# JakobHavtorn/benchmarking-lvms

Measured on AMD Instinct MI355X. Metric: audio frames/sec training (VRNN, 16 kHz mu-law), higher is better.
Workload: dtype f32

## Files before the change

### benchmarking-lvms_amd/csrc/pchain.h

```cpp
#pragma once
#include <algorithm>
#include <cstdlib>

#include "common.h"

namespace blvm {
namespace pchain {

constexpr unsigned SENTINEL = 0xFFFFFFFFu;
constexpr unsigned SPIN_LIMIT = 1u << 22;

typedef unsigned u32x4 __attribute__((ext_vector_type(4)));
typedef __amdgpu_buffer_rsrc_t rsrc_t;
constexpr int AUX_SC1 = 16;
#ifndef PCHAIN_POLL_AUX
#define PCHAIN_POLL_AUX AUX_SC1
#endif
#ifndef PCHAIN_STORE_AUX
#define PCHAIN_STORE_AUX AUX_SC1
#endif
__device__ __forceinline__ rsrc_t make_rsrc(const void* base) {
  const unsigned long long u = reinterpret_cast<unsigned long long>(base);
  const unsigned lo = (unsigned)__builtin_amdgcn_readfirstlane((int)(unsigned)u), hi = (unsigned)__builtin_amdgcn_readfirstlane((int)(unsigned)(u >> 32));
  return __builtin_amdgcn_make_buffer_rsrc(reinterpret_cast<void*>(((unsigned long long)hi << 32) | lo), 0, 0xFFFFFFFFu, 0x00020000);
}
__device__ __forceinline__ f32x4 ld_sc1_x4(rsrc_t r, unsigned byte_off) {
  return __builtin_bit_cast(f32x4, __builtin_amdgcn_raw_buffer_load_b128(r, (int)byte_off, 0, PCHAIN_POLL_AUX));
}
__device__ __forceinline__ float ld_sc1(rsrc_t r, unsigned byte_off) {
  return __builtin_bit_cast(float, __builtin_amdgcn_raw_buffer_load_b32(r, (int)byte_off, 0, PCHAIN_POLL_AUX));
}
__device__ __forceinline__ void st_sc1(rsrc_t r, unsigned byte_off, float v) {
  __builtin_amdgcn_raw_buffer_store_b32(__builtin_bit_cast(unsigned, v), r, (int)byte_off, 0, PCHAIN_STORE_AUX);
}

__device__ __forceinline__ bool is_sentinel(float x) { return __float_as_uint(x) == SENTINEL; }
__device__ __forceinline__ bool any_sentinel(const f32x4& v) {
  return is_sentinel(v[0]) | is_sentinel(v[1]) | is_sentinel(v[2]) | is_sentinel(v[3]);
}

struct Ctl {
  unsigned* dev;
  unsigned* host;
  unsigned epoch;
  __device__ __forceinline__ bool aborted() const { return __hip_atomic_load(dev, __ATOMIC_RELAXED, __HIP_MEMORY_SCOPE_AGENT) == epoch; }
  __device__ __forceinline__ void abort(unsigned code) const {
    if (__hip_atomic_exchange(dev, epoch, __ATOMIC_RELAXED, __HIP_MEMORY_SCOPE_AGENT) != epoch) {
      __hip_atomic_store(host + 1, code, __ATOMIC_RELAXED, __HIP_MEMORY_SCOPE_SYSTEM);
      __hip_atomic_fetch_add(host, 1u, __ATOMIC_RELAXED, __HIP_MEMORY_SCOPE_SYSTEM);
    }
  }
};

__device__ __forceinline__ bool spin_tick(unsigned& spins, const Ctl& ctl, unsigned code, bool& dead) {
  ++spins;
  if ((spins & 255u) == 0) {
    if (ctl.aborted()) { dead = true; return true; }
    if (spins >= SPIN_LIMIT) { ctl.abort(code); dead = true; return true; }
  }
  return false;
}

struct Poll {
  Ctl ctl;
  unsigned code;
  bool dead;
  int nap;
#ifdef PCHAIN_TPROF
  unsigned long long t_first = 0, t_ok = 0, t_end = 0, tp[8] = {0, 0, 0, 0, 0, 0, 0, 0};
  unsigned polls = 0;
#endif
  __device__ __forceinline__ void sleep() const {
    if (nap > 8) __builtin_amdgcn_s_sleep(32);
    else __builtin_amdgcn_s_sleep(1);
  }
};

struct MapSame { static constexpr int of(int) { return 0; } static constexpr bool sum = false; };
struct MapId { static constexpr int of(int g) { return g; } static constexpr bool sum = false; };
struct MapPairs { static constexpr int of(int g) { return g >> 1; } static constexpr bool sum = false; };
struct MapSum { static constexpr int of(int) { return 0; } static constexpr bool sum = true; };

struct NoMid {
  __device__ __forceinline__ void operator()() const {}
};

typedef short s16x4 __attribute__((ext_vector_type(4)));
typedef unsigned u32x2 __attribute__((ext_vector_type(2)));
typedef float f32x2_t __attribute__((ext_vector_type(2)));
typedef __bf16 bf16x2_t __attribute__((ext_vector_type(2)));
typedef _Float16 f16x2_t __attribute__((ext_vector_type(2)));
typedef _Float16 f16x4_t __attribute__((ext_vector_type(4)));
__device__ __forceinline__ unsigned pk_bf16(float a, float b) {
  return __builtin_bit_cast(unsigned, __builtin_convertvector((f32x2_t){a, b}, bf16x2_t));
}
template <int OT>
__device__ __forceinline__ unsigned pk16(float a, float b) {
  if constexpr (OT == OP_F16) return __builtin_bit_cast(unsigned, __builtin_convertvector((f32x2_t){a, b}, f16x2_t));
  else return pk_bf16(a, b);
}
template <int OT>
__device__ __forceinline__ f32x4 mfma16(s16x4 a, s16x4 b, f32x4 acc) {
  if constexpr (OT == OP_F16)
    return __builtin_amdgcn_mfma_f32_16x16x16f16(__builtin_bit_cast(f16x4_t, a), __builtin_bit_cast(f16x4_t, b), acc, 0, 0, 0);
  else return __builtin_amdgcn_mfma_f32_16x16x16bf16_1k(a, b, acc, 0, 0, 0);
}
template <int OT> struct WFrag { typedef u32x2 type; };
template <> struct WFrag<OP_F32> { typedef f32x4 type; };

template <int NW, int OT, int GA, int G, class AMap, int CH, class Mid>
__device__ __forceinline__ void mgemm_trip(const rsrc_t (&ar)[GA], unsigned aoff, const float* const (&ap)[GA], const char* const (&wp)[G], int kc,
                                           bool aok, bool polled, f32x4 (&acc)[G], Poll& pl, Mid& mid, bool& mid_pending) {
  constexpr int STEP = NW * 16;
  typedef typename WFrag<OT>::type wfrag;
  constexpr int ES = OT != OP_F32 ? 2 : 4;
  wfrag w[G][CH];
  f32x4 a[GA][CH];
#pragma unroll
  for (int u = 0; u < CH; ++u)
#pragma unroll
    for (int g = 0; g < G; ++g) w[g][u] = *reinterpret_cast<const wfrag*>(wp[g] + (size_t)ES * 16 * (size_t)(kc + u * STEP));
  if (!polled) {
#pragma unroll
    for (int u = 0; u < CH; ++u)
#pragma unroll
      for (int g = 0; g < GA; ++g) a[g][u] = *reinterpret_cast<const f32x4*>(ap[g] + kc + u * STEP);
    if (mid_pending) { mid(); mid_pending = false; }
  } else {
    unsigned spins = 0;
    for (;;) {
#pragma unroll
      for (int u = 0; u < CH; ++u)
#pragma unroll
        for (int g = 0; g < GA; ++g) a[g][u] = ld_sc1_x4(ar[g], aoff + 64u * (unsigned)(kc + u * STEP));
      if (mid_pending) { mid(); mid_pending = false; }
      bool bad = false;
#pragma unroll
      for (int u = 0; u < CH; ++u)
#pragma unroll
        for (int g = 0; g < GA; ++g) bad |= any_sentinel(a[g][u]);
#ifdef PCHAIN_TPROF
      if (spins == 0 && pl.t_first == 0) pl.t_first = wall_clock64();
      pl.polls++;
#endif
      if (!__any(bad && aok) || pl.dead) break;
      if (spin_tick(spins, pl.ctl, pl.code, pl.dead)) break;
      pl.sleep();
    }
#ifdef PCHAIN_TPROF
    pl.t_ok = wall_clock64();
#endif
  }
  if constexpr (AMap::sum) {
#pragma unroll
    for (int u = 0; u < CH; ++u)
#pragma unroll
      for (int ga = 1; ga < GA; ++ga) a[0][u] += a[ga][u];
  }
  if constexpr (OT != OP_F32) {
#pragma unroll
    for (int u = 0; u < CH; ++u) {
      s16x4 ab[GA];
#pragma unroll
      for (int ga = 0; ga < GA; ++ga) {
        const f32x4 x = a[ga][u];
        const u32x2 q = {aok ? pk16<OT>(x[0], x[1]) : 0u, aok ? pk16<OT>(x[2], x[3]) : 0u};
        ab[ga] = __builtin_bit_cast(s16x4, q);
      }
#pragma unroll
      for (int g = 0; g < G; ++g) acc[g] = mfma16<OT>(ab[AMap::of(g)], __builtin_bit_cast(s16x4, w[g][u]), acc[g]);
    }
  } else {
#pragma unroll
    for (int u = 0; u < CH; ++u)
#pragma unroll
      for (int e = 0; e < 4; ++e)
#pragma unroll
        for (int g = 0; g < G; ++g) acc[g] = __builtin_amdgcn_mfma_f32_16x16x4f32(aok ? a[AMap::of(g)][u][e] : 0.f, w[g][u][e], acc[g], 0, 0, 0);
  }
}

template <int NW, int OT, int GA, int G, class AMap, class Mid = NoMid>
__device__ __forceinline__ void mgemm16(const float* const (&A)[GA], const int (&lda)[GA], bool polled, int r0, int nrows,
                                        const float* const (&W)[G], const int (&c0)[G], int K, f32x4 (&acc)[G], Poll& pl, Mid mid = Mid(),
                                        int a_width = 0, int w_width = 0) {
  constexpr int STEP = NW * 16;
  constexpr int FR = (NW >= 16 ? 6 : 12) / (G + GA);
  constexpr int MAXCH = FR >= 6 ? 6 : (FR >= 4 ? 4 : (FR >= 2 ? 2 : 1));
  const int lane = threadIdx.x & 63, wave = threadIdx.x >> 6;
  const int rr = lane & 15, q = lane >> 4;
  const bool aok = (r0 + rr) < nrows;
  rsrc_t ar[GA];
  const float* ap[GA];
  const char* wp[G];
#pragma unroll
  for (int g = 0; g < GA; ++g) {
    ar[g] = make_rsrc(A[g]);
    ap[g] = A[g] + (size_t)(aok ? r0 + rr : r0) * (polled ? 0 : lda[g]) + 4 * q;
  }
  const unsigned aoff = 4u * ((unsigned)(r0 >> 4) * 16u * (unsigned)(a_width > 0 ? a_width : K) + 4u * (unsigned)lane);
#pragma unroll
  for (int g = 0; g < G; ++g) wp[g] = reinterpret_cast<const char*>(W[g]) + (OT != OP_F32 ? 2 : 4) * ((size_t)c0[g] * (w_width > 0 ? w_width : K) + 4 * lane);
  int nch = (K / 16 - wave + NW - 1) / NW;
  int kc = wave * 16;
  bool mid_pending = true;
  if constexpr (MAXCH >= 6) for (; nch >= 6; nch -= 6, kc += 6 * STEP) mgemm_trip<NW, OT, GA, G, AMap, 6>(ar, aoff, ap, wp, kc, aok, polled, acc, pl, mid, mid_pending);
  if constexpr (MAXCH >= 4) for (; nch >= 4; nch -= 4, kc += 4 * STEP) mgemm_trip<NW, OT, GA, G, AMap, 4>(ar, aoff, ap, wp, kc, aok, polled, acc, pl, mid, mid_pending);
  if constexpr (MAXCH >= 2) for (; nch >= 2; nch -= 2, kc += 2 * STEP) mgemm_trip<NW, OT, GA, G, AMap, 2>(ar, aoff, ap, wp, kc, aok, polled, acc, pl, mid, mid_pending);
  for (; nch >= 1; nch -= 1, kc += STEP) mgemm_trip<NW, OT, GA, G, AMap, 1>(ar, aoff, ap, wp, kc, aok, polled, acc, pl, mid, mid_pending);
  if (mid_pending) mid();
}

template <int N>
__device__ __forceinline__ void poll_words(const rsrc_t (&r)[N], const unsigned (&off)[N], float (&v)[N], bool need, Poll& pl) {
  unsigned spins = 0;
  for (;;) {
#pragma unroll
    for (int i = 0; i < N; ++i) v[i] = ld_sc1(r[i], off[i]);
    bool bad = false;
#pragma unroll
    for (int i = 0; i < N; ++i) bad |= is_sentinel(v[i]);
    if (!__any(bad && need) || pl.dead) break;
    if (spin_tick(spins, pl.ctl, pl.code, pl.dead)) break;
    pl.sleep();
  }
}

__device__ __forceinline__ int first_tile(int w, int wg0, int nwg, int ntiles) {
  return (w >= wg0 && w < wg0 + nwg) ? w - wg0 : ntiles;
}

struct TileIter {
  int rt, ct, j, step, x, n;
  bool xcd;
  __host__ __device__ __forceinline__ TileIter(int w, int wg0, int nwg, int rt_, int ct_, bool xcd_) : rt(rt_), ct(ct_), xcd(xcd_) {
    const int wl = w - wg0;
    const bool in = w >= wg0 && wl < nwg;
    if (xcd) {
      x = wl & 7; step = nwg >> 3; j = wl >> 3;
      n = x < ct ? ((ct - x + 7) >> 3) * rt : 0;
    } else {
      x = 0; step = nwg; j = wl;
      n = rt * ct;
    }
    if (!in || step < 1) { j = 0; n = 0; step = 1; x = 0; }
  }
  __host__ __device__ __forceinline__ bool valid() const { return j < n; }
  __host__ __device__ __forceinline__ void next() { j += step; }
  __host__ __device__ __forceinline__ int r0() const { return (j % rt) * 16; }
  __host__ __device__ __forceinline__ int c() const { return xcd ? x + 8 * (j / rt) : j / rt; }
};

inline int tiles_per_workgroup(int rt, int ct, int nwg, bool xcd) {
  if (nwg <= 0) return 0;
  if (xcd) return nwg >= 8 ? (((ct + 7) / 8) * rt + nwg / 8 - 1) / (nwg / 8) : ((ct + 7) / 8) * rt;
  return (ct * rt + nwg - 1) / nwg;
}

__device__ __forceinline__ void canary_wait(const float* A16, int r0, int K, Poll& pl, int a_width = 0) {
  if (threadIdx.x < 64) {
    const int lane = threadIdx.x, np = K >> 4;
    const rsrc_t r = make_rsrc(A16 + (size_t)(r0 >> 4) * 16 * (a_width > 0 ? a_width : K));
    unsigned spins = 0;
    for (;;) {
      bool bad = false;
      for (int p0 = 0; p0 < np; p0 += 64) {
        const int pr = p0 + lane;
        const float v = ld_sc1(r, 1024u * (unsigned)(pr < np ? pr : 0));
        bad |= (pr < np) && is_sentinel(v);
      }
      if (!__any(bad) || pl.dead) break;
      if (spin_tick(spins, pl.ctl, pl.code, pl.dead)) break;
      pl.sleep();
    }
  }
  __syncthreads();
}

struct WMem {
  static constexpr bool resident = false;
  static constexpr int products = 0;
};
template <int OT, int G, int NCH>
struct WRegs {
  static constexpr bool resident = true;
  static constexpr int products = G;
  typename WFrag<OT>::type w[G][NCH];
};
template <int NW, int OT, int G, int NCH>
__device__ __forceinline__ void load_w(typename WFrag<OT>::type (&w)[G][NCH], const float* const* W, const int (&c0)[G], int ldw) {
  typedef typename WFrag<OT>::type wfrag;
  const int lane = threadIdx.x & 63, wave = threadIdx.x >> 6;
  constexpr int ES = OT != OP_F32 ? 2 : 4;
#pragma unroll
  for (int g = 0; g < G; ++g) {
    const char* base = reinterpret_cast<const char*>(W[g]) + (size_t)ES * ((size_t)c0[g] * ldw + 4 * lane);
#pragma unroll
    for (int u = 0; u < NCH; ++u) w[g][u] = *reinterpret_cast<const wfrag*>(base + (size_t)ES * 256 * (size_t)(wave + u * NW));
  }
}
template <int NW, int OT, int GA, int G, class AMap, int NCH, bool SHARED, class Mid>
__device__ __forceinline__ void product_regs(const float* const (&A16)[GA], int r0, int nrows, int width,
                                             const typename WFrag<OT>::type (&w)[G][NCH], f32x4 (&acc)[G], Poll& pl, Mid mid) {
  static_assert(!SHARED || GA == 1, "the shared-slab form reads one operand");
  const int lane = threadIdx.x & 63, wave = threadIdx.x >> 6;
  const bool aok = (r0 + (lane & 15)) < nrows;
  rsrc_t ar[GA];
#pragma unroll
  for (int g = 0; g < GA; ++g) ar[g] = make_rsrc(A16[g]);
  const unsigned aoff = 4u * ((unsigned)(r0 >> 4) * 16u * (unsigned)width + 4u * (unsigned)lane) + 1024u * (unsigned)wave;
  f32x4 a[GA][NCH];
  unsigned spins = 0;
  bool mid_pending = true;
  if constexpr (SHARED) {
    canary_wait(A16[0], r0, width, pl);
    const float* ap = A16[0] + (size_t)(r0 >> 4) * 16 * width + 4 * lane + 256 * wave;
#pragma unroll
    for (int u = 0; u < NCH; ++u) a[0][u] = *reinterpret_cast<const f32x4*>(ap + 256 * (size_t)(u * NW));
    mid();
    mid_pending = false;
    bool bad = false;
#pragma unroll
    for (int u = 0; u < NCH; ++u) bad |= any_sentinel(a[0][u]);
    if (!__any(bad && aok)) goto multiply;
  }
  for (;;) {
#pragma unroll
    for (int u = 0; u < NCH; ++u)
#pragma unroll
      for (int g = 0; g < GA; ++g) a[g][u] = ld_sc1_x4(ar[g], aoff + 1024u * (unsigned)(u * NW));
    if (mid_pending) { mid(); mid_pending = false; }
    bool bad = false;
#pragma unroll
    for (int u = 0; u < NCH; ++u)
#pragma unroll
      for (int g = 0; g < GA; ++g) bad |= any_sentinel(a[g][u]);
    if (!__any(bad && aok) || pl.dead) break;
    if (spin_tick(spins, pl.ctl, pl.code, pl.dead)) break;
    pl.sleep();
  }
multiply:
  if constexpr (AMap::sum) {
#pragma unroll
    for (int u = 0; u < NCH; ++u)
#pragma unroll
      for (int ga = 1; ga < GA; ++ga) a[0][u] += a[ga][u];
  }
  if constexpr (OT != OP_F32) {
#pragma unroll
    for (int u = 0; u < NCH; ++u) {
      s16x4 ab[GA];
#pragma unroll
      for (int ga = 0; ga < GA; ++ga) {
        const f32x4 x = a[ga][u];
        const u32x2 q = {aok ? pk16<OT>(x[0], x[1]) : 0u, aok ? pk16<OT>(x[2], x[3]) : 0u};
        ab[ga] = __builtin_bit_cast(s16x4, q);
      }
#pragma unroll
      for (int g = 0; g < G; ++g) acc[g] = mfma16<OT>(ab[AMap::of(g)], __builtin_bit_cast(s16x4, w[g][u]), acc[g]);
    }
  } else {
#pragma unroll
    for (int u = 0; u < NCH; ++u)
#pragma unroll
      for (int e = 0; e < 4; ++e)
#pragma unroll
        for (int g = 0; g < G; ++g) acc[g] = __builtin_amdgcn_mfma_f32_16x16x4f32(aok ? a[AMap::of(g)][u][e] : 0.f, w[g][u][e], acc[g], 0, 0, 0);
  }
}

template <int NW, int OT, int GA, int G, class AMap, class Mid = NoMid>
__device__ __forceinline__ void tile_product(const WMem&, const float* const (&A)[GA], const int (&lda)[GA], bool polled, int r0, int nrows,
                                             const float* const (&W)[G], const int (&c0)[G], int K, f32x4 (&acc)[G], Poll& pl, Mid mid = Mid(),
                                             int a_width = 0, int w_width = 0) {
  mgemm16<NW, OT, GA, G, AMap>(A, lda, polled, r0, nrows, W, c0, K, acc, pl, mid, a_width, w_width);
}
template <int NW, int OT, int GA, int G, class AMap, class Mid = NoMid, int NCH>
__device__ __forceinline__ void tile_product(const WRegs<OT, G, NCH>& ws, const float* const (&A)[GA], const int (&)[GA], bool, int r0, int nrows,
                                             const float* const (&)[G], const int (&)[G], int, f32x4 (&acc)[G], Poll& pl, Mid mid = Mid(),
                                             int a_width = 0, int = 0) {
  product_regs<NW, OT, GA, G, AMap, NCH, false>(A, r0, nrows, a_width > 0 ? a_width : NCH * 16 * NW, ws.w, acc, pl, mid);
}

struct Out {
  float* rm;
  int ld;
  bool rm_sc1;
  float* x16;
  int n16;
  float* x16b = nullptr;
  int n16b = 0;
};
__device__ __forceinline__ Out out_rm(float* p, int ld, bool sc1 = false) { return Out{p, ld, sc1, nullptr, 0}; }
__device__ __forceinline__ Out out_both(float* p, int ld, float* x16, int n16, bool sc1 = false) { return Out{p, ld, sc1, x16, n16}; }
__device__ __forceinline__ void put(const Out& o, int r0, int c0, int row, int col, float x) {
  if (o.rm != nullptr) {
    if (o.rm_sc1) st_sc1(make_rsrc(o.rm), 4u * ((unsigned)row * (unsigned)o.ld + (unsigned)col), x);
    else o.rm[(size_t)row * o.ld + col] = x;
  }
  const int rr = row - r0, cc = col - c0;
  const unsigned in_block = (unsigned)((rr + 16 * ((cc & 15) >> 2)) * 4 + (cc & 3));
  if (o.x16 != nullptr) st_sc1(make_rsrc(o.x16), 4u * ((((unsigned)(r0 >> 4) * (unsigned)o.n16 + (unsigned)((c0 + cc) >> 4)) << 8) + in_block), x);
  if (o.x16b != nullptr) st_sc1(make_rsrc(o.x16b), 4u * ((((unsigned)(r0 >> 4) * (unsigned)o.n16b + (unsigned)((c0 + cc) >> 4)) << 8) + in_block), x);
}


struct LinLate {
  const float *bias, *add, *gate;
  int ldadd, ldgate;
  bool add_polled, relu;
  float slope;
  Out out;
};
template <int NW, int OT, class Late, class WS = WMem>
__device__ __forceinline__ void tile_lin_late(const float* A, int lda, bool a_polled, const float* W, int K, Late& late, int r0, int c0, int B,
                                              float* red, Poll& pl, const float* A2 = nullptr, const float* A3 = nullptr, int w_width = 0,
                                              const WS& ws = WS()) {
  const int t = threadIdx.x & 255;
  const int row = r0 + (t >> 4), col = c0 + (t & 15);
  const bool own = threadIdx.x < 256 && row < B;
  const int rowc = row < B ? row : r0;
#ifdef PCHAIN_TPROF
  const unsigned long long t0 = wall_clock64();
  pl.t_first = 0; pl.polls = 0;
#endif
  float e_bias = 0.f, e_gate = 1.f, e_add = 0.f;
  LinLate L;
  auto prefetch = [&]() {
    L = late();
    if (L.bias) e_bias = L.bias[col];
    if (L.gate) e_gate = L.gate[(size_t)rowc * L.ldgate + col];
    if (L.add && !L.add_polled) e_add = L.add[(size_t)rowc * L.ldadd + col];
  };
  f32x4 acc[1] = {{0.f, 0.f, 0.f, 0.f}};
  if (A2 != nullptr) {
    const float* const As[3] = {A, A2, A3};
    const float* const Ws[1] = {W};
    const int la[3] = {0, 0, 0}, cs[1] = {c0};
    tile_product<NW, OT, 3, 1, MapSum>(ws, As, la, true, r0, B, Ws, cs, K, acc, pl, prefetch, lda, w_width);
  } else {
    const float* const As[1] = {A};
    const float* const Ws[1] = {W};
    const int la[1] = {lda}, cs[1] = {c0};
    tile_product<NW, OT, 1, 1, MapSame>(ws, As, la, a_polled, r0, B, Ws, cs, K, acc, pl, prefetch, a_polled ? lda : 0, w_width);
  }
  float v[1];
  reduce_tiles<1, NW>(acc, red, v);
#ifdef PCHAIN_TPROF
  if (a_polled && pl.nap == 1) {
    const unsigned long long t3 = wall_clock64();
    pl.tp[0] += 1; pl.tp[1] += pl.t_first - t0; pl.tp[2] += pl.t_ok - pl.t_first; pl.tp[3] += t3 - pl.t_ok; pl.tp[4] += pl.polls;
    if (pl.t_end != 0) pl.tp[6] += t0 - pl.t_end;
  }
#endif
  if (threadIdx.x >= 256) return;
  if (L.add && L.add_polled) {
    const rsrc_t rs[1] = {make_rsrc(L.add)};
    const unsigned os[1] = {4u * ((unsigned)rowc * (unsigned)L.ldadd + (unsigned)col)};
    float ws[1];
    poll_words<1>(rs, os, ws, own, pl);
    e_add = ws[0];
  }
  if (!own) return;
  float x = v[0] + e_bias + e_add;
  if (L.relu) x = x > 0.f ? x : x * L.slope;
  if (L.gate) x = e_gate > 0.f ? x : x * L.slope;
  put(L.out, r0, c0, row, col, x);
#ifdef PCHAIN_TPROF
  if (a_polled && pl.nap == 1) { pl.t_end = wall_clock64(); }
#endif
}
template <int NW, int OT = OP_F32>
__device__ __forceinline__ void tile_lin(const float* A, int lda, bool a_polled, const float* W, int K, const float* bias,
                                         const float* add, int ldadd, bool add_polled, const float* gate, int ldgate, bool relu,
                                         float slope, const Out& out, int r0, int c0, int B, float* red, Poll& pl) {
  auto late = [&]() { return LinLate{bias, add, gate, ldadd, ldgate, add_polled, relu, slope, out}; };
  tile_lin_late<NW, OT>(A, lda, a_polled, W, K, late, r0, c0, B, red, pl);
}

struct HeadOut {
  float *mu_p, *sd_p, *mu_q, *sd_q, *raw_p, *raw_q, *muq_raw;
  Out z;
};
template <int NW, int OT = OP_F32, class WS = WMem>
__device__ __forceinline__ void tile_head(const float* P, const float* Q, bool polled, const float* Wp, const float* bp, const float* Wq,
                                          const float* bq, const float* eps, const HeadOut& o, int H, int Z, int residual, float beta,
                                          float inv_beta, float sd_eps, int r0, int c0, int B, float* red, Poll& pl, const WS& ws = WS()) {
  const int t = threadIdx.x & 255;
  const int row = r0 + (t >> 4), col = c0 + (t & 15);
  const bool own = threadIdx.x < 256 && row < B;
  const size_t oc = (size_t)(row < B ? row : r0) * Z + col;
  float b0 = 0.f, b1 = 0.f, b2 = 0.f, b3 = 0.f, e = 0.f;
  auto prefetch = [&]() { b0 = bp[col]; b1 = bp[Z + col]; b2 = bq[col]; b3 = bq[Z + col]; e = eps[oc]; };
  f32x4 acc[4];
#pragma unroll
  for (int g = 0; g < 4; ++g) acc[g] = (f32x4){0.f, 0.f, 0.f, 0.f};
  {
    const float* const As[2] = {P, Q};
    const float* const Ws[4] = {Wp, Wp, Wq, Wq};
    const int la[2] = {H, H}, cs[4] = {c0, Z + c0, c0, Z + c0};
    tile_product<NW, OT, 2, 4, MapPairs>(ws, As, la, polled, r0, B, Ws, cs, H, acc, pl, prefetch);
  }
  float v[4];
  reduce_tiles<4, NW>(acc, red, v);
  if (!own) return;
  const size_t oo = (size_t)row * Z + col;
  const float mp = v[0] + b0, rp = v[1] + b1, rq = v[3] + b3;
  float mq = v[2] + b2;
  const float sp = softplus_beta(rp, beta, inv_beta) + sd_eps;
  const float sq = softplus_beta(rq, beta, inv_beta) + sd_eps;
  if (o.muq_raw != nullptr) o.muq_raw[oo] = mq;
  float sqc = sq;
  if (residual == 1) {
    mq += mp;
  } else if (residual == 2) {
    const float pq = 1.f / (sq * sq), pp = 1.f / (sp * sp);
    const float var = 1.f / (pq + pp);
    mq = var * (mq * pq + mp * pp);
    sqc = sqrtf(var);
  } else if (residual == 3) {
    mq = mp;
    sqc = sp;
  }
  put(o.z, r0, c0, row, col, e * sqc + mq);
  o.mu_p[oo] = mp; o.sd_p[oo] = sp; o.mu_q[oo] = mq; o.sd_q[oo] = sqc;
  o.raw_p[oo] = rp; o.raw_q[oo] = rq;
}

template <int NW, int OT = OP_F32, class WS = WMem>
__device__ __forceinline__ void tile_gru(const float* X, int ldx, bool polled, const float* Wih, int K, const float* xg, const float* bih,
                                         const float* gh, const float* hprev, int ldh, int R, const Out& hnew, float* rg, float* ug, float* ng,
                                         int r0, int c0, int B, float* red, Poll& pl, const WS& ws = WS()) {
  const int t = threadIdx.x & 255;
  const int row = r0 + (t >> 4), col = c0 + (t & 15);
  const bool own = threadIdx.x < 256 && row < B;
  const int rowc = row < B ? row : r0;
  const size_t o3 = (size_t)rowc * 3 * R + col;
  const rsrc_t rgh = make_rsrc(gh), rhp = make_rsrc(hprev);
  const rsrc_t ps[4] = {rgh, rgh, rgh, rhp};
  const unsigned po[4] = {4u * (unsigned)o3, 4u * (unsigned)(o3 + R), 4u * (unsigned)(o3 + 2 * R), 4u * ((unsigned)rowc * (unsigned)ldh + (unsigned)col)};
  float w[4] = {0.f, 0.f, 0.f, 0.f}, x0 = 0.f, x1 = 0.f, x2 = 0.f;
  auto prefetch = [&]() {
#pragma unroll
    for (int i = 0; i < 4; ++i) w[i] = ld_sc1(ps[i], po[i]);
    x0 = (xg ? xg[o3] : 0.f) + (bih ? bih[col] : 0.f);
    x1 = (xg ? xg[o3 + R] : 0.f) + (bih ? bih[R + col] : 0.f);
    x2 = (xg ? xg[o3 + 2 * R] : 0.f) + (bih ? bih[2 * R + col] : 0.f);
  };
  f32x4 acc[3];
#pragma unroll
  for (int g = 0; g < 3; ++g) acc[g] = (f32x4){0.f, 0.f, 0.f, 0.f};
  {
    const float* const As[1] = {X};
    const float* const Ws[3] = {Wih, Wih, Wih};
    const int la[1] = {ldx}, cs[3] = {c0, R + c0, 2 * R + c0};
    tile_product<NW, OT, 1, 3, MapSame>(ws, As, la, polled, r0, B, Ws, cs, K, acc, pl, prefetch);
  }
  float v[3];
  reduce_tiles<3, NW>(acc, red, v);
  if (threadIdx.x >= 256) return;
  if (__any(own && (is_sentinel(w[0]) | is_sentinel(w[1]) | is_sentinel(w[2]) | is_sentinel(w[3])))) poll_words<4>(ps, po, w, own, pl);
  if (!own) return;
  const float r = sigmoidf_(v[0] + x0 + w[0]);
  const float u = sigmoidf_(v[1] + x1 + w[1]);
  const float n = tanhf(v[2] + x2 + r * w[2]);
  put(hnew, r0, c0, row, col, (1.f - u) * n + u * w[3]);
  const size_t o = (size_t)row * R + col;
  rg[o] = r; ug[o] = u; ng[o] = n;
}

struct DzIn {
  const float *mu_q, *sd_q, *mu_p, *sd_p, *eps, *raw_q, *raw_p, *muq_raw;
  const int32_t* x_sl;
  const float *c_raw, *c_fn;
  int t, stride, residual;
  float fn_floor, beta, sd_eps;
  bool has_gemm = true;
};
template <int NW, int OT = OP_F32, class WS = WMem>
__device__ __forceinline__ void tile_dz(const float* D, const float* WT, const float* D2, const float* WT2, bool polled, const float* dz_add,
                                        int ld_add, bool add_polled, const DzIn& a, const Out& dqh, const Out& dph, int H, int Z, int r0, int c0,
                                        int B, float* red, Poll& pl, const WS& ws = WS()) {
  const int t = threadIdx.x & 255;
  const int row = r0 + (t >> 4), col = c0 + (t & 15);
  const bool own = threadIdx.x < 256 && row < B;
  const int rowc = row < B ? row : r0;
  const size_t o = (size_t)rowc * Z + col;
  float mq = 0.f, sq = 1.f, mp = 0.f, sp = 1.f, e = 0.f, rq = 0.f, rp = 0.f, c_raw = 0.f, c_fn = 0.f, e_add = 0.f;
  auto prefetch = [&]() {
    mq = a.mu_q[o]; sq = a.sd_q[o]; mp = a.mu_p[o]; sp = a.sd_p[o]; e = a.eps[o]; rq = a.raw_q[o]; rp = a.raw_p[o];
    if (a.c_fn != nullptr || a.c_raw != nullptr) {
      const bool live = (long long)a.t * a.stride < a.x_sl[rowc];
      c_raw = (live && a.c_raw != nullptr) ? a.c_raw[rowc] : 0.f;
      c_fn = (live && a.c_fn != nullptr) ? a.c_fn[rowc] : 0.f;
    }
    if (dz_add != nullptr && !add_polled) e_add = dz_add[(size_t)rowc * ld_add + col];
  };
  float v[2] = {0.f, 0.f};
  if (a.has_gemm) {
    f32x4 acc[2];
    acc[0] = (f32x4){0.f, 0.f, 0.f, 0.f};
    acc[1] = (f32x4){0.f, 0.f, 0.f, 0.f};
    if (WS::products != 1 && D2 != nullptr) {
      if constexpr (WS::products != 1) {
        const float* const As[2] = {D, D2};
        const float* const Ws[2] = {WT, WT2};
        const int la[2] = {H, H}, cs[2] = {c0, c0};
        tile_product<NW, OT, 2, 2, MapId>(ws, As, la, polled, r0, B, Ws, cs, H, acc, pl, prefetch);
      }
    } else {
      if constexpr (WS::products != 2) {
        f32x4 a1[1] = {acc[0]};
        const float* const As[1] = {D};
        const float* const Ws[1] = {WT};
        const int la[1] = {H}, cs[1] = {c0};
        tile_product<NW, OT, 1, 1, MapSame>(ws, As, la, polled, r0, B, Ws, cs, H, a1, pl, prefetch);
        acc[0] = a1[0];
      }
    }
    reduce_tiles<2, NW>(acc, red, v);
  } else {
    prefetch();
  }
  if (threadIdx.x >= 256) return;
  if (dz_add != nullptr && add_polled) {
    const rsrc_t rs[1] = {make_rsrc(dz_add)};
    const unsigned os[1] = {4u * ((unsigned)rowc * (unsigned)ld_add + (unsigned)col)};
    float ws[1];
    poll_words<1>(rs, os, ws, own, pl);
    e_add = ws[0];
  }
  if (!own) return;
  const float dz = v[0] + v[1] + e_add;
  const float d = mq - mp, ip2 = 1.f / (sp * sp);
  float coef = c_raw;
  if (c_fn != 0.f) {
    const float k = logf(sp) - logf(sq) + (sq * sq + d * d) * 0.5f * ip2 - 0.5f;
    if (!(a.fn_floor > 0.f) || k > a.fn_floor) coef += c_fn;
  }
  float g_muq = dz + coef * d * ip2;
  float g_sdq = dz * e + coef * (sq * ip2 - 1.f / sq);
  float g_mup = -coef * d * ip2;
  float g_sdp = coef * (1.f / sp - (sq * sq + d * d) * ip2 / sp);
  if (a.residual == 1) {
    g_mup += g_muq;
  } else if (a.residual == 2) {
    const float mqr = a.muq_raw[o];
    const float sqr = softplus_beta(rq, a.beta, 1.f / a.beta) + a.sd_eps;
    const float pq = 1.f / (sqr * sqr), pp = ip2, var = sq * sq;
    const float half_s3 = 0.5f * var * sq;
    const float g_pq = g_muq * var * (mqr - mq) - g_sdq * half_s3;
    const float g_pp = g_muq * var * (mp - mq) - g_sdq * half_s3;
    g_mup += g_muq * var * pp;
    g_sdp += g_pp * (-2.f * pp / sp);
    g_sdq = g_pq * (-2.f * pq / sqr);
    g_muq = g_muq * var * pq;
  }
  put(dqh, r0, c0, row, col, g_muq);
  put(dqh, r0, Z + c0, row, Z + col, g_sdq * sigmoidf_(a.beta * rq));
  put(dph, r0, c0, row, col, g_mup);
  put(dph, r0, Z + c0, row, Z + col, g_sdp * sigmoidf_(a.beta * rp));
}

struct GrubIn {
  const float *D0, *D1, *W0, *W1, *g_in, *g_add;
  const float *rg, *ug, *ng, *gh, *hprev, *dd;
  int ldh, ld_gadd;
  Out dgi, dgh;
  float *ga, *g_out;
  bool has_gemm, has_gin, has_gates;
};
template <int NW, int OT = OP_F32, class WS = WMem>
__device__ __forceinline__ void tile_grub(const GrubIn& a, int K, int R, int r0, int c0, int B, float* red, Poll& pl, const WS& ws = WS()) {
  const int tt = threadIdx.x & 255;
  const int row = r0 + (tt >> 4), col = c0 + (tt & 15);
  const bool own = threadIdx.x < 256 && row < B;
  const int rowc = row < B ? row : r0;
  const size_t o = (size_t)rowc * R + col, o3 = (size_t)rowc * 3 * R + col;
  float r = 0.f, u = 0.f, n = 0.f, hn = 0.f, hp = 0.f, dd = 0.f, gadd = 0.f, g0 = 0.f;
  auto prefetch = [&]() {
    if (a.has_gin) g0 = ld_sc1(make_rsrc(a.g_in), 4u * (unsigned)o);
    if (a.has_gates) {
      r = a.rg[o]; u = a.ug[o]; n = a.ng[o]; hn = a.gh[o3 + 2 * R];
      hp = a.hprev[(size_t)rowc * a.ldh + col];
      if (a.dd != nullptr) dd = a.dd[(size_t)rowc * a.ldh + col];
    }
    if (a.g_add != nullptr) gadd = a.g_add[(size_t)rowc * a.ld_gadd + col];
  };
  float v[2] = {0.f, 0.f};
  if (!a.has_gemm) prefetch();
  if (a.has_gemm) {
    f32x4 acc[2];
    acc[0] = (f32x4){0.f, 0.f, 0.f, 0.f};
    acc[1] = (f32x4){0.f, 0.f, 0.f, 0.f};
    const float* const As[2] = {a.D0, a.D1};
    const float* const Ws[2] = {a.W0, a.W1};
    const int la[2] = {0, 0}, cs[2] = {c0, c0};
    tile_product<NW, OT, 2, 2, MapId>(ws, As, la, true, r0, B, Ws, cs, K, acc, pl, prefetch);
    reduce_tiles<2, NW>(acc, red, v);
  }
  if (threadIdx.x >= 256) return;
  if (a.has_gin && __any(own && is_sentinel(g0))) {
    const rsrc_t rs[1] = {make_rsrc(a.g_in)};
    const unsigned os[1] = {4u * (unsigned)o};
    float ws[1];
    poll_words<1>(rs, os, ws, own, pl);
    g0 = ws[0];
  }
  if (!own) return;
  const float g = (g0 + gadd) + v[0] + v[1];
  if (!a.has_gates) { a.g_out[(size_t)row * R + col] = g; return; }
  const float dn_pre = g * (1.f - u) * (1.f - n * n);
  const float du_pre = g * (hp - n) * u * (1.f - u);
  const float dr_pre = dn_pre * hn * r * (1.f - r);
  put(a.dgi, r0, c0, row, col, dr_pre); put(a.dgi, r0, R + c0, row, R + col, du_pre); put(a.dgi, r0, 2 * R + c0, row, 2 * R + col, dn_pre);
  put(a.dgh, r0, c0, row, col, dr_pre); put(a.dgh, r0, R + c0, row, R + col, du_pre); put(a.dgh, r0, 2 * R + c0, row, 2 * R + col, dn_pre * r);
  st_sc1(make_rsrc(a.ga), 4u * ((unsigned)row * (unsigned)R + (unsigned)col), g * u + dd);
}

__device__ __forceinline__ int seq_time_index(int j, int reverse, const int32_t* lens, int row) {
  if (!reverse) return j;
  const int n = lens[row];
  return j < n ? n - 1 - j : j;
}
struct GruSeqIn {
  const float *H16, *Whh, *bhh;
  const float* xg;
  const int32_t* lens;
  const float* hprev;
  float* out;
  float *rg, *ug, *ng, *ghn;
  long out_ts;
  int out_ld, j, reverse;
};
template <int NW, int OT = OP_F32>
__device__ __forceinline__ void tile_gru_seq(const GruSeqIn& a, const Out& hnext, int R, int r0, int c0, int B, float* red, Poll& pl) {
  const int t = threadIdx.x & 255;
  const int row = r0 + (t >> 4), col = c0 + (t & 15);
  const bool own = threadIdx.x < 256 && row < B;
  const int rowc = row < B ? row : r0;
  const size_t o = (size_t)rowc * R + col;
  int idx = 0;
  float x0 = 0.f, x1 = 0.f, x2 = 0.f, b0 = 0.f, b1 = 0.f, b2 = 0.f, hp = 0.f;
  auto prefetch = [&]() {
    idx = seq_time_index(a.j, a.reverse, a.lens, rowc);
    const size_t ox = ((size_t)idx * B + rowc) * 3 * R + col;
    x0 = a.xg[ox]; x1 = a.xg[ox + R]; x2 = a.xg[ox + 2 * R];
    b0 = a.bhh[col]; b1 = a.bhh[R + col]; b2 = a.bhh[2 * R + col];
    hp = a.hprev[o];
  };
  f32x4 acc[3];
#pragma unroll
  for (int g = 0; g < 3; ++g) acc[g] = (f32x4){0.f, 0.f, 0.f, 0.f};
  {
    const float* const As[1] = {a.H16};
    const float* const Ws[3] = {a.Whh, a.Whh, a.Whh};
    const int la[1] = {0}, cs[3] = {c0, R + c0, 2 * R + c0};
    mgemm16<NW, OT, 1, 3, MapSame>(As, la, true, r0, B, Ws, cs, R, acc, pl, prefetch);
  }
  float v[3];
  reduce_tiles<3, NW>(acc, red, v);
  if (!own) return;
  const float hn = v[2] + b2;
  const float r = sigmoidf_(x0 + v[0] + b0);
  const float u = sigmoidf_(x1 + v[1] + b1);
  const float n = tanhf(x2 + r * hn);
  const float h2 = (1.f - u) * n + u * hp;
  put(hnext, r0, c0, row, col, h2);
  a.out[(size_t)idx * a.out_ts + (size_t)row * a.out_ld + col] = h2;
  a.rg[o] = r; a.ug[o] = u; a.ng[o] = n; a.ghn[o] = hn;
}

struct GruSeqBwdIn {
  const float *DGHn16, *WhhT;
  const float* dout;
  const float *rg, *ug, *ng, *ghn, *hprev;
  const int32_t* lens;
  float* G;
  float* DGI;
  float* dh0;
  long out_ts;
  int out_ld, j, reverse;
  bool has_gemm, has_gates;
};
template <int NW, int OT = OP_F32>
__device__ __forceinline__ void tile_gru_seq_bwd(const GruSeqBwdIn& a, const Out& dgh, int R, int r0, int c0, int B, float* red, Poll& pl) {
  const int t = threadIdx.x & 255;
  const int row = r0 + (t >> 4), col = c0 + (t & 15);
  const bool own = threadIdx.x < 256 && row < B;
  const int rowc = row < B ? row : r0;
  const size_t o = (size_t)rowc * R + col;
  float g = 0.f, dout = 0.f, r = 0.f, u = 0.f, n = 0.f, hn = 0.f, hp = 0.f;
  int idx = 0;
  auto prefetch = [&]() {
    g = a.G[o];
    if (a.has_gates) {
      idx = seq_time_index(a.j, a.reverse, a.lens, rowc);
      dout = a.dout[(size_t)idx * a.out_ts + (size_t)rowc * a.out_ld + col];
      r = a.rg[o]; u = a.ug[o]; n = a.ng[o]; hn = a.ghn[o]; hp = a.hprev[o];
    }
  };
  float v[1] = {0.f};
  if (a.has_gemm) {
    f32x4 acc[1] = {{0.f, 0.f, 0.f, 0.f}};
    const float* const As[1] = {a.DGHn16};
    const float* const Ws[1] = {a.WhhT};
    const int la[1] = {0}, cs[1] = {c0};
    mgemm16<NW, OT, 1, 1, MapSame>(As, la, true, r0, B, Ws, cs, 3 * R, acc, pl, prefetch);
    reduce_tiles<1, NW>(acc, red, v);
  } else {
    prefetch();
    __syncthreads();
  }
  if (!own) return;
  g += dout + v[0];
  if (!a.has_gates) { a.dh0[o] = g; return; }
  const float dn_pre = g * (1.f - u) * (1.f - n * n);
  const float du_pre = g * (hp - n) * u * (1.f - u);
  const float dr_pre = dn_pre * hn * r * (1.f - r);
  const size_t oi = ((size_t)idx * B + row) * 3 * R + col;
  a.DGI[oi] = dr_pre; a.DGI[oi + R] = du_pre; a.DGI[oi + 2 * R] = dn_pre;
  put(dgh, r0, c0, row, col, dr_pre);
  put(dgh, r0, R + c0, row, R + col, du_pre);
  put(dgh, r0, 2 * R + c0, row, 2 * R + col, dn_pre * r);
  a.G[o] = g * u;
}

struct LstmSeqIn {
  const float *H16, *Whh, *bhh;
  const float* xg;
  const int32_t* lens;
  const float *hprev, *cprev;
  float *cnext, *out, *gates;
  int t;
};
template <int NW, int OT = OP_F32>
__device__ __forceinline__ void tile_lstm_seq(const LstmSeqIn& a, const Out& hnext, int H, int r0, int c0, int B, float* red, Poll& pl) {
  const int tt = threadIdx.x & 255;
  const int row = r0 + (tt >> 4), col = c0 + (tt & 15);
  const bool own = threadIdx.x < 256 && row < B;
  const int rowc = row < B ? row : r0;
  const size_t o = (size_t)rowc * H + col, o4 = (size_t)rowc * 4 * H + col;
  float x0 = 0.f, x1 = 0.f, x2 = 0.f, x3 = 0.f, hp = 0.f, cp = 0.f;
  bool live = true;
  auto prefetch = [&]() {
    x0 = a.xg[o4] + a.bhh[col]; x1 = a.xg[o4 + H] + a.bhh[H + col];
    x2 = a.xg[o4 + 2 * H] + a.bhh[2 * H + col]; x3 = a.xg[o4 + 3 * H] + a.bhh[3 * H + col];
    hp = a.hprev[o]; cp = a.cprev[o];
    live = a.lens == nullptr || a.t < a.lens[rowc];
  };
  f32x4 acc[4];
#pragma unroll
  for (int g = 0; g < 4; ++g) acc[g] = (f32x4){0.f, 0.f, 0.f, 0.f};
  {
    const float* const As[1] = {a.H16};
    const float* const Ws[4] = {a.Whh, a.Whh, a.Whh, a.Whh};
    const int la[1] = {0}, cs[4] = {c0, H + c0, 2 * H + c0, 3 * H + c0};
    mgemm16<NW, OT, 1, 4, MapSame>(As, la, true, r0, B, Ws, cs, H, acc, pl, prefetch);
  }
  float v[4];
  reduce_tiles<4, NW>(acc, red, v);
  if (!own) return;
  const float i = sigmoidf_(v[0] + x0), f = sigmoidf_(v[1] + x1), g = tanhf(v[2] + x2), og = sigmoidf_(v[3] + x3);
  const float c2 = f * cp + i * g;
  const float h2 = og * tanhf(c2);
  a.cnext[o] = live ? c2 : cp;
  put(hnext, r0, c0, row, col, live ? h2 : hp);
  a.out[o] = live ? h2 : 0.f;
  a.gates[o4] = live ? i : 0.f;
  a.gates[o4 + H] = live ? f : 0.f;
  a.gates[o4 + 2 * H] = live ? g : 0.f;
  a.gates[o4 + 3 * H] = live ? og : 0.f;
}

struct LstmSeqBwdIn {
  const float *DGn16, *WhhT;
  const float *dout, *gates, *c_s, *c_s1;
  float* DC;
  float* dh0;
  bool has_gemm, has_gates;
};
template <int NW, int OT = OP_F32>
__device__ __forceinline__ void tile_lstm_seq_bwd(const LstmSeqBwdIn& a, const Out& dg, int H, int r0, int c0, int B, float* red, Poll& pl) {
  const int tt = threadIdx.x & 255;
  const int row = r0 + (tt >> 4), col = c0 + (tt & 15);
  const bool own = threadIdx.x < 256 && row < B;
  const int rowc = row < B ? row : r0;
  const size_t o = (size_t)rowc * H + col, o4 = (size_t)rowc * 4 * H + col;
  float dh = 0.f, ig = 0.f, fg = 0.f, gg = 0.f, og = 0.f, cs = 0.f, cs1 = 0.f, dc = 0.f;
  auto prefetch = [&]() {
    if (a.has_gates) {
      dh = a.dout[o];
      ig = a.gates[o4]; fg = a.gates[o4 + H]; gg = a.gates[o4 + 2 * H]; og = a.gates[o4 + 3 * H];
      cs = a.c_s[o]; cs1 = a.c_s1[o]; dc = a.DC[o];
    }
  };
  float v[1] = {0.f};
  if (a.has_gemm) {
    f32x4 acc[1] = {{0.f, 0.f, 0.f, 0.f}};
    const float* const As[1] = {a.DGn16};
    const float* const Ws[1] = {a.WhhT};
    const int la[1] = {0}, cs_[1] = {c0};
    mgemm16<NW, OT, 1, 1, MapSame>(As, la, true, r0, B, Ws, cs_, 4 * H, acc, pl, prefetch);
    reduce_tiles<1, NW>(acc, red, v);
  } else {
    prefetch();
    __syncthreads();
  }
  if (!own) return;
  dh += v[0];
  if (!a.has_gates) { a.dh0[o] = dh; return; }
  const float tc = tanhf(cs1);
  const float d_o = dh * tc;
  const float dct = dc + dh * og * (1.f - tc * tc);
  put(dg, r0, c0, row, col, dct * gg * ig * (1.f - ig));
  put(dg, r0, H + c0, row, H + col, dct * cs * fg * (1.f - fg));
  put(dg, r0, 2 * H + c0, row, 2 * H + col, dct * ig * (1.f - gg * gg));
  put(dg, r0, 3 * H + c0, row, 3 * H + col, d_o * og * (1.f - og));
  a.DC[o] = dct * fg;
}

template <int NW>
__device__ __forceinline__ void tile_dmol_sample(const float* dec, int ldd, const float* Wl, const float* bl, const float* u, const float* v, int S, int F,
                                                 int num_mix, float log_eps, const Out& xo, int r0, int s0, int B, float* lds, Poll& pl) {
  static_assert(NW == 8 || NW == 16, "waves");
  const int tid = threadIdx.x, wave = tid >> 6, lane = tid & 63;
  float* in = lds;
  float* outp = lds + 16 * 4 * F;
  const int rowlen = 4 * F;
  const int pieces = 16 * rowlen / 4;
  const rsrc_t rd = make_rsrc(dec);
  {
    unsigned spins = 0;
    for (;;) {
      bool bad = false;
      for (int q = tid; q < pieces; q += NW * 64) {
        const int rr = q / (rowlen / 4), cq = q % (rowlen / 4);
        const bool ok = r0 + rr < B;
        const f32x4 x = ld_sc1_x4(rd, 4u * ((unsigned)(ok ? r0 + rr : r0) * (unsigned)ldd + (unsigned)(s0 * F + 4 * cq)));
        bad |= ok && any_sentinel(x);
        *reinterpret_cast<f32x4*>(in + rr * rowlen + 4 * cq) = x;
      }
      if (!__any(bad) || pl.dead) break;
      if (spin_tick(spins, pl.ctl, pl.code, pl.dead)) break;
      pl.sleep();
    }
  }
  __syncthreads();
  {
    const int rr = lane >> 2, ss = lane & 3;
    const float* a = in + rr * rowlen + ss * F;
    if (wave * 4 < F) {
      float acc[4];
#pragma unroll
      for (int j = 0; j < 4; ++j) {
        const int jj = wave * 4 + j;
        acc[j] = jj < F ? bl[jj] : 0.f;
      }
      for (int k = 0; k < F; ++k) {
        const float ak = a[k];
#pragma unroll
        for (int j = 0; j < 4; ++j) {
          const int jj = wave * 4 + j;
          if (jj < F) acc[j] = fmaf(Wl[jj * F + k], ak, acc[j]);
        }
      }
#pragma unroll
      for (int j = 0; j < 4; ++j)
        if (wave * 4 + j < F) outp[lane * 32 + wave * 4 + j] = acc[j];
    }
  }
  __syncthreads();
  if (wave == 0) {
    const int rr = lane >> 2, ss = lane & 3, row = r0 + rr, smp = s0 + ss;
    if (row < B) {
      const float* p = outp + lane * 32;
      const size_t f = (size_t)row * S + smp;
      int best = 0;
      float bv = -INFINITY;
      for (int m = 0; m < num_mix; ++m) {
        float sc = p[m];
        if (u != nullptr) sc -= logf(-logf(u[f * num_mix + m]));
        if (sc > bv) { bv = sc; best = m; }
      }
      const float loc = p[num_mix + best], raw = p[2 * num_mix + best];
      float x = loc;
      if (v != nullptr) {
        const float vv = v[f];
        x = loc + expf(fmaxf(raw, log_eps)) * (logf(vv) - logf(1.f - vv));
        x = fminf(fmaxf(x, -1.f), 1.f);
      }
      put(xo, r0, s0 & ~15, row, smp, x);
    }
  }
  __syncthreads();
}

enum Kind : int { K_LIN = 0, K_HEAD = 1, K_GRU = 2, K_DZ = 3, K_GRUB = 4, K_DMOLS = 5, K_GRUS = 6, K_GRUSB = 7, K_LSTMS = 8, K_LSTMSB = 9, K_LINSEQ = 10 };
enum DescFlag : int {
  DF_RELU = 1,
  DF_A_PLAIN = 2,
  DF_ADD_POLLED = 4,
  DF_RM_SC1 = 8,
  DF_GENTLE = 16,
  DF_CANARY = 32,
  DF_A_SUM3 = 64,
  DF_SEQ_GATE = 128,
};
enum : int { LD_OUT = 3, N16_OUT = 0, N16_OUTB = 1 };
enum : int { LIN_A, LIN_W, LIN_BIAS, LIN_ADD, LIN_GATE, LIN_ORM, LIN_O16, LIN_O16B, LIN_A2, LIN_A3, LIN_LD_A = 0, LIN_LD_ADD = 1, LIN_LD_GATE = 2,
             LIN_I_W_WIDTH = 0, LIN_F_SLOPE = 0 };
enum : int { LINSEQ_A0 = 0, LINSEQ_W = 1, LINSEQ_AUX = 5, LINSEQ_ORM = 9, LINSEQ_O16 = 13, LINSEQ_ADD0 = 17, LINSEQ_LD_ORM = 0,
             LINSEQ_I_LD_ADD0 = 0, LINSEQ_I_N = 1, LINSEQ_I_LD_GATE = 2, LINSEQ_I_K0 = 3, LINSEQ_F_SLOPE = 0 };
enum : int { HEAD_P16, HEAD_Q16, HEAD_WP, HEAD_BP, HEAD_WQ, HEAD_BQ, HEAD_EPS, HEAD_MU_P, HEAD_SD_P, HEAD_MU_Q, HEAD_SD_Q, HEAD_RAW_P, HEAD_RAW_Q,
             HEAD_MUQ_RAW, HEAD_Z, HEAD_Z16, HEAD_Z16B, HEAD_I_Z = 0, HEAD_I_RESIDUAL = 1, HEAD_F_BETA = 0, HEAD_F_INV_BETA = 1, HEAD_F_SD_EPS = 2 };
enum : int { GRU_X16, GRU_WIH, GRU_XG, GRU_GH, GRU_HPREV, GRU_HRM, GRU_H16, GRU_RG, GRU_UG, GRU_NG, GRU_BIH, GRU_H16B, GRU_LD_HPREV = 0, GRU_I_R = 0 };
enum : int { DZ_D16, DZ_WT, DZ_D2_16, DZ_WT2, DZ_ADD, DZ_MU_Q, DZ_SD_Q, DZ_MU_P, DZ_SD_P, DZ_EPS, DZ_RAW_Q, DZ_RAW_P, DZ_MUQ_RAW, DZ_X_SL, DZ_C_RAW,
             DZ_C_FN, DZ_DQH, DZ_DQH16, DZ_DPH, DZ_DPH16, DZ_LD_ADD = 1, DZ_I_Z = 0, DZ_I_RESIDUAL = 1, DZ_I_STRIDE = 2, DZ_I_T0 = 3,
             DZ_F_FN_FLOOR = 0, DZ_F_BETA = 1, DZ_F_SD_EPS = 2, DZ_F_GEMM_FROM = 3 };
enum : int { GRUB_D0_16, GRUB_D1_16, GRUB_W0, GRUB_W1, GRUB_G_IN, GRUB_RG, GRUB_UG, GRUB_NG, GRUB_GH, GRUB_HPREV, GRUB_DD, GRUB_DGI, GRUB_DGI16,
             GRUB_DGH, GRUB_DGH16, GRUB_GA, GRUB_G_OUT, GRUB_G_ADD, GRUB_LD_H = 0, GRUB_LD_GADD = 1, GRUB_I_R = 0, GRUB_I_GEMM_FROM = 1,
             GRUB_I_GATES_TO = 2, GRUB_I_GIN_FROM = 3 };
enum : int { DMOLS_DEC, DMOLS_W, DMOLS_B, DMOLS_U, DMOLS_V, DMOLS_X, DMOLS_X16, DMOLS_LD_DEC = 0, DMOLS_I_S = 0, DMOLS_I_F = 1, DMOLS_I_NMIX = 2,
             DMOLS_F_LOG_EPS = 0 };
enum : int { GRUS_H16, GRUS_WHH, GRUS_BHH, GRUS_XG, GRUS_LENS, GRUS_HPREV, GRUS_HNEXT, GRUS_HNEXT16, GRUS_OUT, GRUS_RG, GRUS_UG, GRUS_NG, GRUS_GHN,
             GRUS_I_R = 0, GRUS_I_REVERSE = 1, GRUS_I_OUT_TS = 2, GRUS_I_OUT_LD = 3 };
enum : int { GRUSB_DGH16_IN, GRUSB_WHHT, GRUSB_DOUT, GRUSB_RG, GRUSB_UG, GRUSB_NG, GRUSB_GHN, GRUSB_HPREV, GRUSB_LENS, GRUSB_G, GRUSB_DGI, GRUSB_DGH,
             GRUSB_DGH16, GRUSB_DH0, GRUSB_N16_T = 1, GRUSB_I_R = 0, GRUSB_I_REVERSE = 1, GRUSB_I_OUT_TS = 2, GRUSB_I_OUT_LD = 3 };
enum : int { LSTMS_H16, LSTMS_WHH, LSTMS_BHH, LSTMS_XG, LSTMS_LENS, LSTMS_HPREV, LSTMS_HNEXT, LSTMS_HNEXT16, LSTMS_CPREV, LSTMS_CNEXT, LSTMS_OUT,
             LSTMS_GATES, LSTMS_I_H = 0 };
enum : int { LSTMSB_DG16_IN, LSTMSB_WHHT, LSTMSB_DOUT, LSTMSB_GATES, LSTMSB_CS, LSTMSB_DC, LSTMSB_DG, LSTMSB_DG16, LSTMSB_DH0, LSTMSB_N16_T = 1, LSTMSB_I_H = 0 };
constexpr int kMaxDesc = 24, kMaxPtr = 20;
struct Desc {
  int kind, ct, wg0, nwg, flags, K, s_begin, s_end;
  int ld[4];
  int n16[2];
  int i[4];
  float f[4];
  unsigned char sidx[kMaxPtr];
  const float* p[kMaxPtr];
};
struct Program {
  int ot = OP_F32;
  int rt_group = 1;
  int s_first = 0;
  int ndesc, S, B, xcd;
  long stride[16];
  Ctl ctl;
  unsigned long long* prof;
  int prof_wg, lds_products;
  Desc d[kMaxDesc];
};

struct Ptr {
  const void* p; long step;
  Ptr(const void* p_ = nullptr, long step_ = 0) : p(p_), step(step_) {}
};
struct Builder {
  Program p{};
  int nstride = 1;
  bool overflow = false;
  void begin(int ot, int S, int B, int lds_products, bool backward, int prof_wg) {
    p.ot = ot; p.S = S; p.B = B; p.xcd = (pchain_tune() & 4) ? 1 : 0; p.lds_products = lds_products;
    p.prof = pchain_profile_buffer() && backward ? pchain_profile_buffer() + 64 : pchain_profile_buffer(); p.prof_wg = prof_wg;
  }
  int stride_index(long v) {
    if (v == 0) return 0;
    for (int i = 1; i < nstride; ++i)
      if (p.stride[i] == v) return i;
    if (nstride >= 16) { overflow = true; return 0; }
    p.stride[nstride] = v;
    return nstride++;
  }
  Desc& add(int kind, int ct, int wg0, int nwg, int K, int flags, int s_begin, int s_end) {
    static Desc dummy;
    if (p.ndesc >= kMaxDesc) { overflow = true; return dummy; }
    Desc& d = p.d[p.ndesc++];
    d = Desc{};
    d.kind = kind; d.ct = ct; d.wg0 = wg0; d.nwg = nwg; d.K = K; d.flags = flags; d.s_begin = s_begin; d.s_end = s_end;
    return d;
  }
  void ptr(Desc& d, int k, Ptr q) {
    d.p[k] = static_cast<const float*>(q.p);
    d.sidx[k] = (unsigned char)(q.p ? stride_index(q.step) : 0);
  }
};
inline Ptr rev(const float* base, long step, long t0) { return Ptr(base ? base + t0 * step : nullptr, -step); }

struct Operands {
  Ptr p[kMaxPtr];
  int ld[4] = {}, n16[2] = {}, i[4] = {}; float f[4] = {};
};
inline Desc& add_desc(Builder& b, int kind, int ct, int wg0, int nwg, int K, int flags, int s_begin, int s_end, const Operands& o) {
  Desc& d = b.add(kind, ct, wg0, nwg, K, flags, s_begin, s_end);
  for (int k = 0; k < kMaxPtr; ++k) b.ptr(d, k, o.p[k]);
  std::copy(o.ld, o.ld + 4, d.ld); std::copy(o.n16, o.n16 + 2, d.n16); std::copy(o.i, o.i + 4, d.i); std::copy(o.f, o.f + 4, d.f);
  return d;
}

struct SeqLink {
  const float *W, *aux;
  float* orm;
  long rm_step;
  int ldo;
  float* o16;
};
inline Desc& add_linseq(Builder& b, int ct, int wg0, int nwg, int K, bool relu, bool gated, int s_begin, int s_end, Ptr A16, int n, const SeqLink* L,
                        long aux_step, long o16_step, int n16, float slope, int ldgate, int K0 = 0, Ptr add0 = Ptr(), int ldadd0 = 0) {
  Desc& d = b.add(K_LINSEQ, ct, wg0, nwg, K, (relu ? DF_RELU : 0) | (gated ? DF_SEQ_GATE : 0), s_begin, s_end);
  b.ptr(d, LINSEQ_A0, A16); b.ptr(d, LINSEQ_ADD0, add0);
  d.i[LINSEQ_I_K0] = (K0 != 0 && K0 != K) ? K0 : 0; d.i[LINSEQ_I_LD_ADD0] = ldadd0;
  for (int i = 0; i < n && i < 4; ++i) {
    b.ptr(d, LINSEQ_W + i, L[i].W); b.ptr(d, LINSEQ_AUX + i, Ptr(L[i].aux, gated ? aux_step : 0)); b.ptr(d, LINSEQ_ORM + i, Ptr(L[i].orm, L[i].rm_step));
    b.ptr(d, LINSEQ_O16 + i, Ptr(L[i].o16, o16_step)); d.ld[LINSEQ_LD_ORM + i] = L[i].ldo;
  }
  if (n > 4) b.overflow = true;
  d.n16[N16_OUT] = n16; d.i[LINSEQ_I_N] = n; d.i[LINSEQ_I_LD_GATE] = ldgate; d.f[LINSEQ_F_SLOPE] = slope;
  return d;
}
inline SeqLink rev_link(const float* W, const float* gate, float* orm, float* o16, long t0, long sB, int ld, long x16) {
  return SeqLink{W, gate ? gate + t0 * sB : nullptr, orm ? orm + t0 * sB : nullptr, -sB, ld, o16 ? o16 + t0 * x16 : nullptr};
}
inline int range_for(int tiles, int avail) { return std::max(8, std::min(avail & ~7, (tiles + 7) & ~7)); }

}

hipError_t pchain_fill_sentinel(void* p, size_t bytes, hipStream_t stream);
inline int pchain_ctl(pchain::Ctl& c) { return pchain_ctl(&c.dev, &c.host, &c.epoch); }
int pchain_prepare(pchain::Builder& bld, const char* who);
int pchain_run(const pchain::Program& prog, hipStream_t stream);
inline int pchain_launch(pchain::Builder& bld, const char* who, hipStream_t stream) {
  BLVM_TRY(pchain_prepare(bld, who));
  return pchain_run(bld.p, stream);
}
int vrnn_launch(pchain::Builder& bld, bool forward, const char* who, hipStream_t stream);
int pchain_rows_to_t16(const float* src, int ld, int B, int K, float* dst, hipStream_t stream, int n16 = 0);
inline int device_cus() {
  static int v = [] {
    int dev = 0, n = 0;
    if (hipGetDevice(&dev) != hipSuccess) return 0;
    if (hipDeviceGetAttribute(&n, hipDeviceAttributeMultiprocessorCount, dev) != hipSuccess) return 0;
    if (const char* e = getenv("BLVM_PCHAIN_CUS")) {
      const int m = atoi(e) & ~7;
      if (m >= 32 && m < n) n = m;
    }
    return n;
  }();
  return v;
}
constexpr int kPchainCarveMaxB = 128;
inline bool pchain_applies(int B) { return B <= pchain_max_batch() && B <= kPchainCarveMaxB; }
inline OpType pchain_optype(int B) { return operand_16bit() && pchain_applies(B) && device_cus() >= 32 ? operand_type() : OP_F32; }

}
```

### benchmarking-lvms_amd/csrc/vrnn_static.h

```cpp
#pragma once
#include <algorithm>
#include <initializer_list>

#include "pchain.h"

namespace blvm {
namespace pchain {

struct LinkRange {
  int ct, wg0, nwg;
};
struct VrnnFwdDeal {
  int def_n, half, g;
  LinkRange hproj, prior, post, head, phi, gru;
};
inline VrnnFwdDeal vrnn_fwd_deal(int ctH, int ctZ, int ctR, int tl, int cus, bool shared) {
  VrnnFwdDeal d;
  d.def_n = shared ? 0 : range_for(3 * ctR * tl, std::min(cus / 4, 64));
  d.half = range_for(ctH * tl, (cus - d.def_n) / 2);
  d.g = 2 * d.half;
  const int wide = shared ? d.half : d.g;
  d.hproj = shared ? LinkRange{3 * ctR, d.half, d.half} : LinkRange{3 * ctR, d.g, d.def_n};
  d.prior = LinkRange{ctH, 0, d.half};
  d.post = LinkRange{ctH, d.half, d.half};
  d.head = LinkRange{ctZ, 0, range_for(ctZ * tl, wide)};
  d.phi = LinkRange{ctH, 0, range_for(ctH * tl, wide)};
  d.gru = LinkRange{ctR, 0, range_for(ctR * tl, d.g)};
  return d;
}
struct VrnnBwdDeal {
  int def_n, half, g, spare;
  bool split3;
  LinkRange grub, part[3], dphi, gb, wide_h, dz, prior, post;
};
inline VrnnBwdDeal vrnn_bwd_deal(int ctH, int ctZ, int ctR, int tl, int cus, bool shared, bool allow_split3) {
  VrnnBwdDeal d;
  d.def_n = shared ? 0 : range_for(ctR * tl, std::min(cus / 4, 64));
  d.half = range_for(ctH * tl, (cus - d.def_n) / 2);
  d.g = 2 * d.half;
  const int wide = shared ? d.half : d.g;
  d.spare = cus - d.g - d.def_n;
  d.split3 = !shared && d.spare >= 8 && d.half >= 8 && allow_split3;
  d.grub = LinkRange{ctR, 0, range_for(ctR * tl, d.g)};
  d.part[0] = LinkRange{ctH, 0, range_for(ctH * tl, d.half)};
  d.part[1] = LinkRange{ctH, d.half, range_for(ctH * tl, d.half)};
  d.part[2] = LinkRange{ctH, d.g + d.def_n, d.split3 ? range_for(ctH * tl, d.spare) : 0};
  d.dphi = LinkRange{ctH, 0, range_for(ctH * tl, wide)};
  d.gb = shared ? LinkRange{ctR, d.half, d.half} : LinkRange{ctR, d.g, d.def_n};
  d.wide_h = LinkRange{ctH, 0, range_for(ctH * tl, wide)};
  d.dz = LinkRange{ctZ, 0, range_for(ctZ * tl, wide)};
  d.prior = LinkRange{ctH, 0, d.half};
  d.post = LinkRange{ctH, d.half, d.half};
  return d;
}

constexpr std::initializer_list<int> kFwdResident = {1, 2, 3, 4, 5};
constexpr std::initializer_list<int> kBwdResident = {0, 1, 2, 3, 5, 6, 7, 8, 9};
inline bool one_tile_each(const Program& p, std::initializer_list<int> links) {
  for (int i : links)
    if (tiles_per_workgroup((p.B + 15) / 16, p.d[i].ct, p.d[i].nwg, p.xcd != 0) > 1) return false;
  return true;
}

}
}
```

### benchmarking-lvms_amd/csrc/vrnn_static.hip

```cpp
#include <algorithm>
#include <mutex>

#include "common.h"
#include "pchain.h"
#include "vrnn_static.h"

namespace blvm {
namespace {
using namespace pchain;

struct SPtr {
  float* base;
  int stride;
  __device__ __forceinline__ float* at(int s) const { return base + (long)s * stride; }
};

constexpr int kMaxTiles = 8;
__device__ __forceinline__ int tile_lanes(int w, int wg0, int nwg, int rt, int ct, bool xcd) {
  TileIter it(w, wg0, nwg, rt, ct, xcd);
  const int lane = threadIdx.x & 63;
  it.j += lane * it.step;
  return (lane < kMaxTiles && it.valid()) ? (it.r0() | (it.c() << 16)) : -1;
}
__device__ __forceinline__ int tile_count(int lanes) { return __popcll(__ballot(lanes >= 0)); }

struct LinChainArgs {
  SPtr a16, orm, o16;
  const float *W, *bias;
  int ldo, n16, B, s0, S, wg0, nwg, ct, xcd;
  Ctl ctl;
};

template <int NW, int K, bool RES>
__global__ __launch_bounds__(NW * 64, 1) void static_lin_chain_kernel(LinChainArgs a) {
  __shared__ __attribute__((aligned(16))) float red[2][NW * 256];
  const int w = blockIdx.x, B = a.B;
  const int tiles = tile_lanes(w, a.wg0, a.nwg, (B + 15) / 16, a.ct, a.xcd != 0);
  const int nt = tile_count(tiles);
  if (nt == 0) return;
  Poll pl{a.ctl, 0u, false, 1};
  int par = 0;
  if constexpr (RES) {
    const int trc = __builtin_amdgcn_readlane(tiles, 0), r0 = trc & 0xffff, c0 = (trc >> 16) * 16;
    WRegs<OP_F32, 1, K / (16 * NW)> ws;
    const float* const Ws[1] = {a.W};
    const int cs[1] = {c0};
    load_w<NW, OP_F32, 1, K / (16 * NW)>(ws.w, Ws, cs, K);
    for (int s = a.s0; s < a.S; ++s) {
      pl.code = (unsigned)s << 4;
      auto late = [&]() { return LinLate{a.bias, nullptr, nullptr, 0, 0, false, true, 0.f, Out{a.orm.at(s), a.ldo, false, a.o16.at(s), a.n16}}; };
      tile_lin_late<NW, OP_F32>(a.a16.at(s), 0, true, a.W, K, late, r0, c0, B, red[par], pl, nullptr, nullptr, 0, ws);
      par ^= 1;
    }
    return;
  }
  for (int s = a.s0; s < a.S; ++s) {
    pl.code = (unsigned)s << 4;
    const float* A = a.a16.at(s);
    auto late = [&]() { return LinLate{a.bias, nullptr, nullptr, 0, 0, false, true, 0.f, Out{a.orm.at(s), a.ldo, false, a.o16.at(s), a.n16}}; };
    for (int tk = 0; tk < nt; ++tk) {
      const int trc = __builtin_amdgcn_readlane(tiles, tk);
      tile_lin_late<NW, false>(A, 0, true, a.W, K, late, trc & 0xffff, (trc >> 16) * 16, B, red[par], pl);
      par ^= 1;
    }
  }
}

constexpr int kH = 256, kR = 512;

struct LinArgs {
  SPtr a, a2, a3, add, gate, orm, o16, o16b;
  const float *W, *bias;
  int ld0, ld1, ld2, ld3, n16, n16b, w_width;
  float slope;
};
struct SeqArgs {
  SPtr a0, add0, aux[4], orm[4], o16[4];
  const float* W[4];
  int ld[4], ldadd0, ldgate, n16;
  float slope;
};
struct HeadArgs {
  SPtr P, Q, eps, mu_p, sd_p, mu_q, sd_q, raw_p, raw_q, muq_raw, z, z16, z16b;
  const float *Wp, *bp, *Wq, *bq;
  int ld3, n16, n16b, Z, residual;
  float beta, inv_beta, sd_eps;
};
struct GruArgs {
  SPtr X, xg, gh, hprev, hrm, h16, h16b, rg, ug, ng;
  const float *Wih, *bih;
  int ld0, ld3, n16, n16b, R;
};
struct DzArgs {
  SPtr D, add, mu_q, sd_q, mu_p, sd_p, eps, raw_q, raw_p, muq_raw, dqh, dqh16, dph, dph16;
  const float *WT, *c_raw, *c_fn;
  const int32_t* x_sl;
  int ld1, ld3, n16, Z, residual, stride, t0, first_gemm;
  float fn_floor, beta, sd_eps;
};
struct GrubArgs {
  SPtr D0, D1, g_in, rg, ug, ng, gh, hprev, dd, dgi, dgi16, dgh, dgh16, ga, g_add;
  const float *W0, *W1, *g_out;
  int ld0, ld1, ld3, n16, R, first_gemm, end_gates, first_gin;
};
struct Deal {
  int wg0, nwg, ct, s_begin, s_end, idx;
};

struct Walk {
  float* red0;
  float* red1;
  int par, B;
  Poll pl;
  __device__ __forceinline__ float* red() { par ^= 1; return par ? red0 : red1; }
  __device__ __forceinline__ void at(const Deal& d, int s, bool gentle, unsigned li = 0) {
    pl.nap = gentle ? 16 : 1;
    pl.code = ((unsigned)s << 4) | (unsigned)d.idx | (li << 28);
  }
};

template <int K, int G = 1>
using Res = WRegs<OP_F32, G, K / 256>;
template <int N, int K0, int K>
struct RunRes {
  Res<K0> first;
  Res<K> rest[N - 1];
};
__device__ __forceinline__ int tile_c0(int tiles) { return (__builtin_amdgcn_readlane(tiles, 0) >> 16) * 16; }

template <int NW, int K>
__device__ __forceinline__ void load_lin(Res<K>& r, const float* W, int ldw, int tiles, int nt) {
  if (nt == 0) return;
  const float* const Ws[1] = {W};
  const int cs[1] = {tile_c0(tiles)};
  load_w<NW, OP_F32, 1, K / 256>(r.w, Ws, cs, ldw > 0 ? ldw : K);
}
template <int NW, int N, int K0, int K>
__device__ __forceinline__ void load_run(RunRes<N, K0, K>& r, const SeqArgs& q, int tiles, int nt) {
  load_lin<NW, K0>(r.first, q.W[0], K0, tiles, nt);
#pragma unroll
  for (int li = 1; li < N; ++li) load_lin<NW, K>(r.rest[li - 1], q.W[li], K, tiles, nt);
}
template <int NW>
__device__ __forceinline__ void load_head(Res<kH, 4>& r, const HeadArgs& q, int tiles, int nt) {
  if (nt == 0) return;
  const int c0 = tile_c0(tiles);
  const float* const Ws[4] = {q.Wp, q.Wp, q.Wq, q.Wq};
  const int cs[4] = {c0, q.Z + c0, c0, q.Z + c0};
  load_w<NW, OP_F32, 4, 1>(r.w, Ws, cs, kH);
}
template <int NW>
__device__ __forceinline__ void load_gru(Res<kH, 3>& r, const GruArgs& q, int tiles, int nt) {
  if (nt == 0) return;
  const int c0 = tile_c0(tiles);
  const float* const Ws[3] = {q.Wih, q.Wih, q.Wih};
  const int cs[3] = {c0, q.R + c0, 2 * q.R + c0};
  load_w<NW, OP_F32, 3, 1>(r.w, Ws, cs, kH);
}
template <int NW>
__device__ __forceinline__ void load_grub(Res<kH, 2>& r, const GrubArgs& q, int tiles, int nt) {
  if (nt == 0) return;
  const int c0 = tile_c0(tiles);
  const float* const Ws[2] = {q.W0, q.W1};
  const int cs[2] = {c0, c0};
  load_w<NW, OP_F32, 2, 1>(r.w, Ws, cs, kH);
}

template <int NW, int K, int FLAGS, class WS>
__device__ __forceinline__ void visit_lin(const LinArgs& q, const Deal& d, int s, int tiles, int nt, Walk& wk, const WS& ws) {
  if (nt == 0 || s < d.s_begin || s >= d.s_end) return;
  constexpr bool sum3 = (FLAGS & DF_A_SUM3) != 0;
  wk.at(d, s, (FLAGS & DF_GENTLE) != 0);
  const float* A = q.a.at(s);
  const float* A2 = sum3 ? q.a2.at(s) : nullptr;
  const float* A3 = sum3 ? q.a3.at(s) : nullptr;
  auto late = [&]() {
    return LinLate{q.bias, q.add.at(s), q.gate.at(s), q.ld1, q.ld2, (FLAGS & DF_ADD_POLLED) != 0, (FLAGS & DF_RELU) != 0, q.slope,
                   Out{q.orm.at(s), q.ld3, (FLAGS & DF_RM_SC1) != 0, q.o16.at(s), q.n16, q.o16b.at(s), q.n16b}};
  };
  for (int tk = 0; tk < (WS::resident ? 1 : nt); ++tk) {
    const int trc = __builtin_amdgcn_readlane(tiles, tk), tr0 = trc & 0xffff, tc0 = (trc >> 16) * 16;
    if constexpr ((FLAGS & DF_CANARY) != 0) canary_wait(A, tr0, K, wk.pl, q.ld0);
    tile_lin_late<NW, OP_F32>(A, q.ld0, true, q.W, K, late, tr0, tc0, wk.B, wk.red(), wk.pl, A2, A3, q.w_width, ws);
  }
}

template <int NW, int N, int K0, int K, bool GATED>
__device__ __forceinline__ void visit_run(const SeqArgs& q, const Deal& d, int s, int tiles, int nt, Walk& wk, const RunRes<N, K0, K>& rr) {
  if (nt == 0 || s < d.s_begin || s >= d.s_end) return;
  const int trc = __builtin_amdgcn_readlane(tiles, 0), tr0 = trc & 0xffff, tc0 = (trc >> 16) * 16;
  const float* A = q.a0.at(s);
#pragma unroll
  for (int li = 0; li < N; ++li) {
    wk.at(d, s, false, (unsigned)li);
    auto late = [&]() {
      const float* aux = q.aux[li].at(s);
      return LinLate{GATED ? nullptr : aux, li == 0 ? q.add0.at(s) : nullptr, GATED ? aux : nullptr, q.ldadd0, q.ldgate, false, !GATED, q.slope,
                     Out{q.orm[li].at(s), q.ld[li], false, q.o16[li].at(s), q.n16}};
    };
    if (li == 0) tile_lin_late<NW, OP_F32>(A, 0, true, q.W[li], K0, late, tr0, tc0, wk.B, wk.red(), wk.pl, nullptr, nullptr, 0, rr.first);
    else tile_lin_late<NW, OP_F32>(A, 0, true, q.W[li], K, late, tr0, tc0, wk.B, wk.red(), wk.pl, nullptr, nullptr, 0, rr.rest[li > 0 ? li - 1 : 0]);
    A = q.o16[li].at(s);
  }
}

template <int NW>
__device__ __forceinline__ void visit_head(const HeadArgs& q, const Deal& d, int s, int tiles, int nt, Walk& wk, const Res<kH, 4>& ws) {
  if (nt == 0 || s < d.s_begin || s >= d.s_end) return;
  wk.at(d, s, false);
  const HeadOut o{q.mu_p.at(s), q.sd_p.at(s), q.mu_q.at(s), q.sd_q.at(s), q.raw_p.at(s), q.raw_q.at(s), q.muq_raw.at(s),
                  Out{q.z.at(s), q.ld3, false, q.z16.at(s), q.n16, q.z16b.at(s), q.n16b}};
  const int trc = __builtin_amdgcn_readlane(tiles, 0);
  tile_head<NW, OP_F32>(q.P.at(s), q.Q.at(s), true, q.Wp, q.bp, q.Wq, q.bq, q.eps.at(s), o, kH, q.Z, q.residual, q.beta, q.inv_beta, q.sd_eps,
                        trc & 0xffff, (trc >> 16) * 16, wk.B, wk.red(), wk.pl, ws);
}

template <int NW>
__device__ __forceinline__ void visit_gru(const GruArgs& q, const Deal& d, int s, int tiles, int nt, Walk& wk, const Res<kH, 3>& ws) {
  if (nt == 0 || s < d.s_begin || s >= d.s_end) return;
  wk.at(d, s, false);
  const Out o{q.hrm.at(s), q.ld3, true, q.h16.at(s), q.n16, q.h16b.at(s), q.n16b};
  const int trc = __builtin_amdgcn_readlane(tiles, 0);
  tile_gru<NW, OP_F32>(q.X.at(s), 0, true, q.Wih, kH, q.xg.at(s), q.bih, q.gh.at(s), q.hprev.at(s), q.ld0, q.R, o, q.rg.at(s), q.ug.at(s), q.ng.at(s),
                       trc & 0xffff, (trc >> 16) * 16, wk.B, wk.red(), wk.pl, ws);
}

template <int NW>
__device__ __forceinline__ void visit_dz(const DzArgs& q, const Deal& d, int s, int tiles, int nt, Walk& wk, const Res<kH>& ws) {
  if (nt == 0 || s < d.s_begin || s >= d.s_end) return;
  wk.at(d, s, false);
  DzIn z;
  z.mu_q = q.mu_q.at(s); z.sd_q = q.sd_q.at(s); z.mu_p = q.mu_p.at(s); z.sd_p = q.sd_p.at(s); z.eps = q.eps.at(s); z.raw_q = q.raw_q.at(s);
  z.raw_p = q.raw_p.at(s); z.muq_raw = q.muq_raw.at(s);
  z.x_sl = q.x_sl; z.c_raw = q.c_raw; z.c_fn = q.c_fn;
  z.t = q.t0 - s; z.stride = q.stride; z.residual = q.residual;
  z.fn_floor = q.fn_floor; z.beta = q.beta; z.sd_eps = q.sd_eps;
  z.has_gemm = s >= q.first_gemm;
  const Out oq{q.dqh.at(s), q.ld3, false, q.dqh16.at(s), q.n16}, op{q.dph.at(s), q.ld3, false, q.dph16.at(s), q.n16};
  const int trc = __builtin_amdgcn_readlane(tiles, 0);
  tile_dz<NW, OP_F32>(q.D.at(s), q.WT, nullptr, nullptr, true, q.add.at(s), q.ld1, false, z, oq, op, kH, q.Z, trc & 0xffff, (trc >> 16) * 16, wk.B,
                      wk.red(), wk.pl, ws);
}

template <int NW>
__device__ __forceinline__ void visit_grub(const GrubArgs& q, const Deal& d, int s, int tiles, int nt, Walk& wk, const Res<kH, 2>& ws) {
  if (nt == 0 || s < d.s_begin || s >= d.s_end) return;
  wk.at(d, s, false);
  GrubIn g;
  g.D0 = q.D0.at(s); g.D1 = q.D1.at(s); g.W0 = q.W0; g.W1 = q.W1; g.g_in = q.g_in.at(s); g.g_add = q.g_add.at(s); g.ld_gadd = q.ld1;
  g.rg = q.rg.at(s); g.ug = q.ug.at(s); g.ng = q.ng.at(s); g.gh = q.gh.at(s); g.hprev = q.hprev.at(s); g.dd = q.dd.at(s); g.ldh = q.ld0;
  g.dgi = Out{q.dgi.at(s), q.ld3, false, q.dgi16.at(s), q.n16};
  g.dgh = Out{q.dgh.at(s), q.ld3, false, q.dgh16.at(s), q.n16};
  g.ga = q.ga.at(s); g.g_out = const_cast<float*>(q.g_out);
  g.has_gemm = s >= q.first_gemm; g.has_gates = s < q.end_gates; g.has_gin = s >= q.first_gin;
  const int trc = __builtin_amdgcn_readlane(tiles, 0);
  tile_grub<NW, OP_F32>(g, kH, q.R, trc & 0xffff, (trc >> 16) * 16, wk.B, wk.red(), wk.pl, ws);
}

template <class A>
__device__ __forceinline__ const A& kargs() {
  typedef const __attribute__((address_space(4))) char kchar;
  kchar* p = (kchar*)__builtin_amdgcn_kernarg_segment_ptr();
  asm volatile("" : "+s"(p));
  return *(const A*)p;
}

struct FwdArgs {
  LinArgs hproj;
  SeqArgs run[2];
  HeadArgs head;
  SeqArgs phi;
  GruArgs gru;
  Deal deal[6];
  int B, s0, S, xcd;
  Ctl ctl;
};
constexpr int kFwdProducts = 4, kBwdProducts = 2;

template <int NW, int HALF>
__device__ __forceinline__ void fwd_half(const FwdArgs& a, int w, int rt, bool xcd, Walk& wk) {
  const int t1 = tile_lanes(w, a.deal[1 + HALF].wg0, a.deal[1 + HALF].nwg, rt, a.deal[1 + HALF].ct, xcd), n1 = tile_count(t1);
  const int t3 = tile_lanes(w, a.deal[3].wg0, a.deal[3].nwg, rt, a.deal[3].ct, xcd), n3 = tile_count(t3);
  const int t4 = tile_lanes(w, a.deal[4].wg0, a.deal[4].nwg, rt, a.deal[4].ct, xcd), n4 = tile_count(t4);
  const int t5 = tile_lanes(w, a.deal[5].wg0, a.deal[5].nwg, rt, a.deal[5].ct, xcd), n5 = tile_count(t5);
  RunRes<3, kR, kH> run;
  Res<kH, 4> head;
  RunRes<4, kH, kH> phi;
  Res<kH, 3> gru;
  load_run<NW>(run, kargs<FwdArgs>().run[HALF], t1, n1);
  load_head<NW>(head, kargs<FwdArgs>().head, t3, n3);
  load_run<NW>(phi, kargs<FwdArgs>().phi, t4, n4);
  load_gru<NW>(gru, kargs<FwdArgs>().gru, t5, n5);
  for (int s = a.s0; s < a.S; ++s) {
    visit_run<NW, 3, kR, kH, false>(kargs<FwdArgs>().run[HALF], kargs<FwdArgs>().deal[1 + HALF], s, t1, n1, wk, run);
    visit_head<NW>(kargs<FwdArgs>().head, kargs<FwdArgs>().deal[3], s, t3, n3, wk, head);
    visit_run<NW, 4, kH, kH, false>(kargs<FwdArgs>().phi, kargs<FwdArgs>().deal[4], s, t4, n4, wk, phi);
    visit_gru<NW>(kargs<FwdArgs>().gru, kargs<FwdArgs>().deal[5], s, t5, n5, wk, gru);
  }
}

template <int NW>
__global__ __launch_bounds__(NW * 64, 1) void vrnn_static_fwd_kernel(FwdArgs a) {
  extern __shared__ __attribute__((aligned(16))) float lds_red[];
  const int w = blockIdx.x, rt = (a.B + 15) / 16;
  const bool xcd = a.xcd != 0;
  Walk wk{lds_red, lds_red + kFwdProducts * NW * 256, 0, a.B, Poll{a.ctl, 0u, false, 1}};
  if (w >= a.deal[0].wg0) {
    const int t0 = tile_lanes(w, a.deal[0].wg0, a.deal[0].nwg, rt, a.deal[0].ct, xcd), n0 = tile_count(t0);
    if (n0 == 0) return;
    for (int s = a.s0; s < a.S; ++s) visit_lin<NW, kR, DF_RM_SC1 | DF_GENTLE | DF_CANARY>(kargs<FwdArgs>().hproj, kargs<FwdArgs>().deal[0], s, t0, n0, wk, WMem());
    return;
  }
  if (w < a.deal[2].wg0) fwd_half<NW, 0>(a, w, rt, xcd, wk);
  else fwd_half<NW, 1>(a, w, rt, xcd, wk);
}

struct BwdArgs {
  GrubArgs grub;
  LinArgs part[3], gb, sum;
  SeqArgs phi;
  DzArgs dz;
  SeqArgs run[2];
  Deal deal[10];
  int B, s0, S, xcd;
  Ctl ctl;
};

template <int NW, int HALF>
__device__ __forceinline__ void bwd_half(const BwdArgs& a, int w, int rt, bool xcd, Walk& wk) {
  const int t0 = tile_lanes(w, a.deal[0].wg0, a.deal[0].nwg, rt, a.deal[0].ct, xcd), n0 = tile_count(t0);
  const int t1 = tile_lanes(w, a.deal[1 + HALF].wg0, a.deal[1 + HALF].nwg, rt, a.deal[1 + HALF].ct, xcd), n1 = tile_count(t1);
  const int t5 = tile_lanes(w, a.deal[5].wg0, a.deal[5].nwg, rt, a.deal[5].ct, xcd), n5 = tile_count(t5);
  const int t6 = tile_lanes(w, a.deal[6].wg0, a.deal[6].nwg, rt, a.deal[6].ct, xcd), n6 = tile_count(t6);
  const int t7 = tile_lanes(w, a.deal[7].wg0, a.deal[7].nwg, rt, a.deal[7].ct, xcd), n7 = tile_count(t7);
  const int t8 = tile_lanes(w, a.deal[8 + HALF].wg0, a.deal[8 + HALF].nwg, rt, a.deal[8 + HALF].ct, xcd), n8 = tile_count(t8);
  Res<kH, 2> grub;
  Res<kR> part;
  Res<kH> sum, dz;
  RunRes<2, kH, kH> phi;
  RunRes<3, 2 * kH, kH> run;
  load_grub<NW>(grub, kargs<BwdArgs>().grub, t0, n0);
  load_lin<NW, kR>(part, kargs<BwdArgs>().part[HALF].W, kargs<BwdArgs>().part[HALF].w_width, t1, n1);
  load_lin<NW, kH>(sum, kargs<BwdArgs>().sum.W, kH, t5, n5);
  load_run<NW>(phi, kargs<BwdArgs>().phi, t6, n6);
  load_lin<NW, kH>(dz, kargs<BwdArgs>().dz.WT, kH, t7, n7);
  load_run<NW>(run, kargs<BwdArgs>().run[HALF], t8, n8);
  for (int s = a.s0; s < a.S; ++s) {
    visit_grub<NW>(kargs<BwdArgs>().grub, kargs<BwdArgs>().deal[0], s, t0, n0, wk, grub);
    visit_lin<NW, kR, 0>(kargs<BwdArgs>().part[HALF], kargs<BwdArgs>().deal[1 + HALF], s, t1, n1, wk, part);
    visit_lin<NW, kH, DF_A_SUM3>(kargs<BwdArgs>().sum, kargs<BwdArgs>().deal[5], s, t5, n5, wk, sum);
    visit_run<NW, 2, kH, kH, true>(kargs<BwdArgs>().phi, kargs<BwdArgs>().deal[6], s, t6, n6, wk, phi);
    visit_dz<NW>(kargs<BwdArgs>().dz, kargs<BwdArgs>().deal[7], s, t7, n7, wk, dz);
    visit_run<NW, 3, 2 * kH, kH, true>(kargs<BwdArgs>().run[HALF], kargs<BwdArgs>().deal[8 + HALF], s, t8, n8, wk, run);
  }
}

template <int NW>
__global__ __launch_bounds__(NW * 64, 1) void vrnn_static_bwd_kernel(BwdArgs a) {
  extern __shared__ __attribute__((aligned(16))) float lds_red[];
  const int w = blockIdx.x, rt = (a.B + 15) / 16;
  const bool xcd = a.xcd != 0;
  Walk wk{lds_red, lds_red + kBwdProducts * NW * 256, 0, a.B, Poll{a.ctl, 0u, false, 1}};
  if (w >= a.deal[3].wg0) {
    const int t = tile_lanes(w, a.deal[3].wg0, a.deal[3].nwg, rt, a.deal[3].ct, xcd), n = tile_count(t);
    if (n == 0) return;
    Res<kR> part;
    load_lin<NW, kR>(part, kargs<BwdArgs>().part[2].W, kargs<BwdArgs>().part[2].w_width, t, n);
    for (int s = a.s0; s < a.S; ++s) visit_lin<NW, kR, 0>(kargs<BwdArgs>().part[2], kargs<BwdArgs>().deal[3], s, t, n, wk, part);
    return;
  }
  if (w >= a.deal[4].wg0) {
    const int t = tile_lanes(w, a.deal[4].wg0, a.deal[4].nwg, rt, a.deal[4].ct, xcd), n = tile_count(t);
    if (n == 0) return;
    for (int s = a.s0; s < a.S; ++s)
      visit_lin<NW, 3 * kR, DF_ADD_POLLED | DF_RM_SC1 | DF_GENTLE | DF_CANARY>(kargs<BwdArgs>().gb, kargs<BwdArgs>().deal[4], s, t, n, wk, WMem());
    return;
  }
  if (w < a.deal[2].wg0) bwd_half<NW, 0>(a, w, rt, xcd, wk);
  else bwd_half<NW, 1>(a, w, rt, xcd, wk);
}

bool int_strides(const Program& p) {
  for (long v : p.stride)
    if (v < -2147483647L || v > 2147483647L) return false;
  return true;
}
SPtr sptr(const Program& p, const Desc& d, int k) { return SPtr{const_cast<float*>(d.p[k]), (int)p.stride[d.sidx[k]]}; }

template <class Kern>
int static_go(Kern kernel, int slot, int grid, size_t lds, const char* what) {
  static std::mutex mu;
  static int attr_dev[3] = {-1, -1, -1}, occ[3] = {0, 0, 0};
  int dev = 0, cus = 0;
  BLVM_HIP(hipGetDevice(&dev));
  BLVM_HIP(hipDeviceGetAttribute(&cus, hipDeviceAttributeMultiprocessorCount, dev));
  {
    std::lock_guard<std::mutex> lock(mu);
    if (attr_dev[slot] != dev) {
      BLVM_HIP(hipFuncSetAttribute(reinterpret_cast<const void*>(kernel), hipFuncAttributeMaxDynamicSharedMemorySize, (int)lds));
      BLVM_HIP(hipOccupancyMaxActiveBlocksPerMultiprocessor(&occ[slot], kernel, 1024, lds));
      attr_dev[slot] = dev;
    }
    BLVM_REQUIRE((long)occ[slot] * cus >= grid, "%s: %d workgroups are not co-resident (%d per CU x %d CUs)", what, grid, occ[slot], cus);
  }
  return BLVM_OK;
}

int static_lin_chain_launch(const Program& p, hipStream_t stream, bool resident) {
  if (p.ndesc != 1 || p.ot != OP_F32 || p.rt_group != 1 || !int_strides(p)) return 1;
  const Desc& d = p.d[0];
  if (d.kind != K_LIN || d.flags != DF_RELU || d.f[LIN_F_SLOPE] != 0.f || (d.K != 256 && d.K != 512) || d.s_begin != 0 || d.s_end != p.S) return 1;
  if (d.ld[LIN_LD_A] != 0 || d.i[LIN_I_W_WIDTH] != 0 || d.p[LIN_ADD] || d.p[LIN_GATE] || d.p[LIN_O16B] || d.p[LIN_A2] || d.p[LIN_A3] || d.n16[N16_OUTB] != 0)
    return 1;
  const int rt = (p.B + 15) / 16;
  if (d.nwg <= 0 || (p.xcd && d.nwg % 8 != 0) || tiles_per_workgroup(rt, d.ct, d.nwg, p.xcd != 0) > (resident ? 1 : kMaxTiles)) return 1;
  LinChainArgs a{sptr(p, d, LIN_A), sptr(p, d, LIN_ORM), sptr(p, d, LIN_O16), d.p[LIN_W], d.p[LIN_BIAS], d.ld[LD_OUT], d.n16[N16_OUT], p.B, p.s_first, p.S,
                 d.wg0, d.nwg, d.ct, p.xcd, p.ctl};
  const int grid = d.wg0 + d.nwg;
  auto go = [&](auto kernel) -> int {
    BLVM_TRY(static_go(kernel, 2, grid, 0, "static_lin_chain"));
    hipLaunchKernelGGL(kernel, dim3(grid), dim3(1024), 0, stream, a);
    BLVM_CHECK_LAUNCH("static_lin_chain");
    return BLVM_OK;
  };
  if (resident) return d.K == 256 ? go(&static_lin_chain_kernel<16, 256, true>) : go(&static_lin_chain_kernel<16, 512, true>);
  return d.K == 256 ? go(&static_lin_chain_kernel<16, 256, false>) : go(&static_lin_chain_kernel<16, 512, false>);
}

int g_static = 1;
long g_static_launches = 0;
bool pchain_static_on() { return g_static != 0; }

SPtr sp(const Program& p, const Desc& d, int k) { return SPtr{const_cast<float*>(d.p[k]), d.p[k] ? (int)p.stride[d.sidx[k]] : 0}; }
Deal deal_of(const Desc& d, int idx) { return Deal{d.wg0, d.nwg, d.ct, d.s_begin, d.s_end, idx}; }
bool within(const Desc& d, int lo, int hi) { return d.wg0 >= lo && d.wg0 + d.nwg <= hi; }
bool few_tiles(const Program& p, const Desc& d) {
  if (d.nwg <= 0 || (p.xcd && d.nwg % 8 != 0)) return false;
  return tiles_per_workgroup((p.B + 15) / 16, d.ct, d.nwg, p.xcd != 0) <= kMaxTiles;
}
bool shaped(const Desc& d, int kind, int flags, int K) { return d.kind == kind && d.flags == flags && d.K == K; }
bool run(const Desc& d, int n, int K0) { return d.i[LINSEQ_I_N] == n && d.i[LINSEQ_I_K0] == K0; }

LinArgs lin_args(const Program& p, const Desc& d) {
  return LinArgs{sp(p, d, LIN_A), sp(p, d, LIN_A2), sp(p, d, LIN_A3), sp(p, d, LIN_ADD), sp(p, d, LIN_GATE), sp(p, d, LIN_ORM), sp(p, d, LIN_O16),
                 sp(p, d, LIN_O16B), d.p[LIN_W], d.p[LIN_BIAS], d.ld[LIN_LD_A], d.ld[LIN_LD_ADD], d.ld[LIN_LD_GATE], d.ld[LD_OUT], d.n16[N16_OUT], d.n16[N16_OUTB],
                 d.i[LIN_I_W_WIDTH], d.f[LIN_F_SLOPE]};
}
SeqArgs seq_args(const Program& p, const Desc& d) {
  SeqArgs q{};
  q.a0 = sp(p, d, LINSEQ_A0); q.add0 = sp(p, d, LINSEQ_ADD0);
  for (int i = 0; i < d.i[LINSEQ_I_N]; ++i) {
    q.W[i] = d.p[LINSEQ_W + i]; q.aux[i] = sp(p, d, LINSEQ_AUX + i); q.orm[i] = sp(p, d, LINSEQ_ORM + i); q.o16[i] = sp(p, d, LINSEQ_O16 + i);
    q.ld[i] = d.ld[LINSEQ_LD_ORM + i];
  }
  q.ldadd0 = d.i[LINSEQ_I_LD_ADD0]; q.ldgate = d.i[LINSEQ_I_LD_GATE]; q.n16 = d.n16[N16_OUT]; q.slope = d.f[LINSEQ_F_SLOPE];
  return q;
}

int vrnn_static_check(const Program& p, int ndesc, int products) {
  if (!pchain_static_on() || p.ndesc != ndesc || p.ot != OP_F32 || p.rt_group != 1 || p.s_first != 0 || p.B > 64) return 1;
  if (p.lds_products != products || !int_strides(p)) return 1;
  for (int i = 0; i < p.ndesc; ++i)
    if (!few_tiles(p, p.d[i])) return 1;
  return 0;
}

int vrnn_static_fwd(const Program& p, hipStream_t stream) {
  if (vrnn_static_check(p, 6, kFwdProducts)) return 1;
  const Desc* d = p.d;
  const int S = p.S;
  for (int i = 0; i < 6; ++i)
    if (d[i].s_begin != 0 || d[i].s_end != S) return 1;
  if (!shaped(d[0], K_LIN, DF_RM_SC1 | DF_GENTLE | DF_CANARY, kR) || !shaped(d[1], K_LINSEQ, DF_RELU, kH) || !shaped(d[2], K_LINSEQ, DF_RELU, kH) ||
      !shaped(d[3], K_HEAD, 0, kH) || !shaped(d[4], K_LINSEQ, DF_RELU, kH) || !shaped(d[5], K_GRU, 0, kH))
    return 1;
  if (!run(d[1], 3, kR) || !run(d[2], 3, kR) || !run(d[4], 4, 0)) return 1;
  if (!one_tile_each(p, kFwdResident)) return 1;
  const int half = d[2].wg0, gentle = d[0].wg0;
  if (d[1].wg0 != 0 || !within(d[1], 0, half) || !within(d[2], half, gentle) || d[0].nwg <= 0) return 1;
  for (int i = 3; i < 6; ++i)
    if (!within(d[i], 0, gentle)) return 1;
  FwdArgs a{};
  a.hproj = lin_args(p, d[0]);
  a.run[0] = seq_args(p, d[1]); a.run[1] = seq_args(p, d[2]); a.phi = seq_args(p, d[4]);
  const Desc &h = d[3], &g = d[5];
  a.head = HeadArgs{sp(p, h, HEAD_P16), sp(p, h, HEAD_Q16), sp(p, h, HEAD_EPS), sp(p, h, HEAD_MU_P), sp(p, h, HEAD_SD_P), sp(p, h, HEAD_MU_Q),
                    sp(p, h, HEAD_SD_Q), sp(p, h, HEAD_RAW_P), sp(p, h, HEAD_RAW_Q), sp(p, h, HEAD_MUQ_RAW), sp(p, h, HEAD_Z), sp(p, h, HEAD_Z16),
                    sp(p, h, HEAD_Z16B), h.p[HEAD_WP], h.p[HEAD_BP], h.p[HEAD_WQ], h.p[HEAD_BQ], h.ld[LD_OUT], h.n16[N16_OUT], h.n16[N16_OUTB],
                    h.i[HEAD_I_Z], h.i[HEAD_I_RESIDUAL], h.f[HEAD_F_BETA], h.f[HEAD_F_INV_BETA], h.f[HEAD_F_SD_EPS]};
  a.gru = GruArgs{sp(p, g, GRU_X16), sp(p, g, GRU_XG), sp(p, g, GRU_GH), sp(p, g, GRU_HPREV), sp(p, g, GRU_HRM), sp(p, g, GRU_H16), sp(p, g, GRU_H16B),
                  sp(p, g, GRU_RG), sp(p, g, GRU_UG), sp(p, g, GRU_NG), g.p[GRU_WIH], g.p[GRU_BIH], g.ld[GRU_LD_HPREV], g.ld[LD_OUT], g.n16[N16_OUT],
                  g.n16[N16_OUTB], g.i[GRU_I_R]};
  int grid = 0;
  for (int i = 0; i < 6; ++i) { a.deal[i] = deal_of(d[i], i); grid = std::max(grid, d[i].wg0 + d[i].nwg); }
  a.B = p.B; a.s0 = p.s_first; a.S = S; a.xcd = p.xcd; a.ctl = p.ctl;
  const size_t lds = sizeof(float) * 2 * kFwdProducts * 16 * 256;
  BLVM_TRY(static_go(&vrnn_static_fwd_kernel<16>, 0, grid, lds, "vrnn_static_fwd"));
  hipLaunchKernelGGL(vrnn_static_fwd_kernel<16>, dim3(grid), dim3(1024), lds, stream, a);
  BLVM_CHECK_LAUNCH("vrnn_static_fwd");
  ++g_static_launches;
  return BLVM_OK;
}

int vrnn_static_bwd(const Program& p, hipStream_t stream) {
  if (vrnn_static_check(p, 10, kBwdProducts)) return 1;
  const Desc* d = p.d;
  const int S = p.S;
  for (int i = 0; i < 10; ++i)
    if (d[i].s_begin != 0 || d[i].s_end != (i == 0 ? S : S - 1)) return 1;
  if (!shaped(d[0], K_GRUB, 0, kH) || !shaped(d[1], K_LIN, 0, kR) || !shaped(d[2], K_LIN, 0, kR) || !shaped(d[3], K_LIN, 0, kR) ||
      !shaped(d[4], K_LIN, DF_ADD_POLLED | DF_RM_SC1 | DF_GENTLE | DF_CANARY, 3 * kR) || !shaped(d[5], K_LIN, DF_A_SUM3, kH) ||
      !shaped(d[6], K_LINSEQ, DF_SEQ_GATE, kH) || !shaped(d[7], K_DZ, 0, kH) || !shaped(d[8], K_LINSEQ, DF_SEQ_GATE, kH) ||
      !shaped(d[9], K_LINSEQ, DF_SEQ_GATE, kH))
    return 1;
  if (!run(d[6], 2, 0) || !run(d[8], 3, 2 * kH) || !run(d[9], 3, 2 * kH)) return 1;
  if (!one_tile_each(p, kBwdResident) || d[7].p[DZ_D2_16] != nullptr) return 1;
  const int half = d[2].wg0, gentle = d[4].wg0, spare = d[3].wg0;
  if (!within(d[1], 0, half) || !within(d[8], 0, half) || !within(d[2], half, gentle) || !within(d[9], half, gentle) || !within(d[4], gentle, spare) ||
      d[3].nwg <= 0)
    return 1;
  for (int i : {0, 5, 6, 7})
    if (!within(d[i], 0, gentle)) return 1;
  BwdArgs a{};
  const Desc& g = d[0];
  a.grub = GrubArgs{sp(p, g, GRUB_D0_16), sp(p, g, GRUB_D1_16), sp(p, g, GRUB_G_IN), sp(p, g, GRUB_RG), sp(p, g, GRUB_UG), sp(p, g, GRUB_NG), sp(p, g, GRUB_GH),
                    sp(p, g, GRUB_HPREV), sp(p, g, GRUB_DD), sp(p, g, GRUB_DGI), sp(p, g, GRUB_DGI16), sp(p, g, GRUB_DGH), sp(p, g, GRUB_DGH16), sp(p, g, GRUB_GA),
                    sp(p, g, GRUB_G_ADD), g.p[GRUB_W0], g.p[GRUB_W1], g.p[GRUB_G_OUT], g.ld[GRUB_LD_H], g.ld[GRUB_LD_GADD], g.ld[LD_OUT], g.n16[N16_OUT],
                    g.i[GRUB_I_R], g.i[GRUB_I_GEMM_FROM], g.i[GRUB_I_GATES_TO], g.i[GRUB_I_GIN_FROM]};
  for (int k = 0; k < 3; ++k) a.part[k] = lin_args(p, d[1 + k]);
  a.gb = lin_args(p, d[4]); a.sum = lin_args(p, d[5]);
  a.phi = seq_args(p, d[6]); a.run[0] = seq_args(p, d[8]); a.run[1] = seq_args(p, d[9]);
  const Desc& z = d[7];
  a.dz = DzArgs{sp(p, z, DZ_D16), sp(p, z, DZ_ADD), sp(p, z, DZ_MU_Q), sp(p, z, DZ_SD_Q), sp(p, z, DZ_MU_P), sp(p, z, DZ_SD_P),
                sp(p, z, DZ_EPS), sp(p, z, DZ_RAW_Q), sp(p, z, DZ_RAW_P), sp(p, z, DZ_MUQ_RAW), sp(p, z, DZ_DQH), sp(p, z, DZ_DQH16), sp(p, z, DZ_DPH),
                sp(p, z, DZ_DPH16), z.p[DZ_WT], z.p[DZ_C_RAW], z.p[DZ_C_FN], reinterpret_cast<const int32_t*>(z.p[DZ_X_SL]), z.ld[DZ_LD_ADD],
                z.ld[LD_OUT], z.n16[N16_OUT], z.i[DZ_I_Z], z.i[DZ_I_RESIDUAL], z.i[DZ_I_STRIDE], z.i[DZ_I_T0], (int)z.f[DZ_F_GEMM_FROM], z.f[DZ_F_FN_FLOOR],
                z.f[DZ_F_BETA], z.f[DZ_F_SD_EPS]};
  int grid = 0;
  for (int i = 0; i < 10; ++i) { a.deal[i] = deal_of(d[i], i); grid = std::max(grid, d[i].wg0 + d[i].nwg); }
  a.B = p.B; a.s0 = p.s_first; a.S = S; a.xcd = p.xcd; a.ctl = p.ctl;
  const size_t lds = sizeof(float) * 2 * kBwdProducts * 16 * 256;
  BLVM_TRY(static_go(&vrnn_static_bwd_kernel<16>, 1, grid, lds, "vrnn_static_bwd"));
  hipLaunchKernelGGL(vrnn_static_bwd_kernel<16>, dim3(grid), dim3(1024), lds, stream, a);
  BLVM_CHECK_LAUNCH("vrnn_static_bwd");
  ++g_static_launches;
  return BLVM_OK;
}

}

int vrnn_launch(pchain::Builder& bld, bool forward, const char* who, hipStream_t stream) {
  BLVM_TRY(pchain_prepare(bld, who));
  const int rc = forward ? vrnn_static_fwd(bld.p, stream) : vrnn_static_bwd(bld.p, stream);
  return rc == 1 ? pchain_run(bld.p, stream) : rc;
}

}

extern "C" int blvm_pchain_static(int mode) {
  if (mode == -2) return (int)std::min<long>(blvm::g_static_launches, 0x7fffffffL);
  const int was = blvm::g_static;
  if (mode >= 0) blvm::g_static = mode != 0;
  return was;
}

static int static_chain_probe(const float* W16, const float* bias, float* x16, float* xs, int B, int N, int L, int nwg, void* stream_, bool resident) {
  using namespace blvm;
  using namespace blvm::pchain;
  hipStream_t s = static_cast<hipStream_t>(stream_);
  BLVM_REQUIRE(W16 && bias && x16 && xs && B > 0 && N > 0 && N % 16 == 0 && L > 0, "pchain_static_chain_probe: bad arguments");
  const int rt = (B + 15) / 16;
  const long x = (long)rt * 16 * N, sN = (long)B * N;
  Builder bld;
  bld.begin(OP_F32, L, B, 1, false, 0);
  const int nw = nwg > 0 ? nwg : range_for((N / 16) * rt, device_cus() & ~7);
  Operands o;
  o.p[LIN_A] = {x16, x}; o.p[LIN_W] = W16; o.p[LIN_BIAS] = bias; o.p[LIN_ORM] = {xs, sN}; o.p[LIN_O16] = {x16 + x, x}; o.ld[LD_OUT] = N; o.n16[N16_OUT] = N / 16;
  add_desc(bld, K_LIN, N / 16, 0, nw, N, DF_RELU, 0, L, o);
  BLVM_HIP(pchain_fill_sentinel(x16 + x, sizeof(float) * (size_t)x * L, s));
  BLVM_TRY(pchain_prepare(bld, "pchain_static_chain_probe"));
  const int rc = static_lin_chain_launch(bld.p, s, resident);
  BLVM_REQUIRE(rc != 1, "pchain_static_chain_probe: no static kernel for N = %d (256, 512) or this deal", N);
  return rc;
}
extern "C" int blvm_pchain_static_chain_probe(const float* W16, const float* bias, float* x16, float* xs, int B, int N, int L, int nwg, void* stream) {
  return static_chain_probe(W16, bias, x16, xs, B, N, L, nwg, stream, true);
}
extern "C" int blvm_pchain_static_chain_probe_fetch(const float* W16, const float* bias, float* x16, float* xs, int B, int N, int L, int nwg, void* stream) {
  return static_chain_probe(W16, bias, x16, xs, B, N, L, nwg, stream, false);
}
```

Measured before the change: 80.56 million.

## Pack head weights, keep gentle-link weights resident, and add static-kernel profiling

The head link now uses half-width column tiles with packed mean/raw weight rows, fetching two weight products instead of four and using a DPP lane shuffle to pair outputs. This doubles the number of head workgroups through a new deal. The gentle links (hproj forward, gb backward) now preload up to a fixed number of weight tiles into registers instead of streaming weights from memory every step. The change also adds scalar-register hints, a single-product reduce path, and optional TPROF timing instrumentation. It raises register pressure and tightens the eligibility checks for the static path, so more shapes may fall back to the generic chain.

```diff
diff --git a/benchmarking-lvms_amd/csrc/pchain.h b/benchmarking-lvms_amd/csrc/pchain.h
--- a/benchmarking-lvms_amd/csrc/pchain.h
+++ b/benchmarking-lvms_amd/csrc/pchain.h
@@ -68,7 +68,8 @@
   int nap;
 #ifdef PCHAIN_TPROF
   unsigned long long t_first = 0, t_ok = 0, t_end = 0, tp[8] = {0, 0, 0, 0, 0, 0, 0, 0};
-  unsigned polls = 0;
+  unsigned long long t_red = 0;
+  unsigned polls = 0, late = 0;
 #endif
   __device__ __forceinline__ void sleep() const {
     if (nap > 8) __builtin_amdgcn_s_sleep(32);
@@ -299,6 +300,19 @@
     for (int u = 0; u < NCH; ++u) w[g][u] = *reinterpret_cast<const wfrag*>(base + (size_t)ES * 256 * (size_t)(wave + u * NW));
   }
 }
+template <int NW, int OT, int G, int NCH>
+__device__ __forceinline__ void load_w_packed(typename WFrag<OT>::type (&w)[G][NCH], const float* const* W, const int (&lo)[G], const int (&hi)[G], int ldw) {
+  typedef typename WFrag<OT>::type wfrag;
+  const int lane = threadIdx.x & 63, wave = threadIdx.x >> 6, j = lane & 15;
+  constexpr int ES = OT != OP_F32 ? 2 : 4;
+#pragma unroll
+  for (int g = 0; g < G; ++g) {
+    const int r = j < 8 ? lo[g] + j : hi[g] + j - 8;
+    const char* base = reinterpret_cast<const char*>(W[g]) + (size_t)ES * ((size_t)(r & ~15) * ldw + 4 * ((r & 15) + (lane & 48)));
+#pragma unroll
+    for (int u = 0; u < NCH; ++u) w[g][u] = *reinterpret_cast<const wfrag*>(base + (size_t)ES * 256 * (size_t)(wave + u * NW));
+  }
+}
 template <int NW, int OT, int GA, int G, class AMap, int NCH, bool SHARED, class Mid>
 __device__ __forceinline__ void product_regs(const float* const (&A16)[GA], int r0, int nrows, int width,
                                              const typename WFrag<OT>::type (&w)[G][NCH], f32x4 (&acc)[G], Poll& pl, Mid mid) {
@@ -335,11 +349,19 @@
     for (int u = 0; u < NCH; ++u)
 #pragma unroll
       for (int g = 0; g < GA; ++g) bad |= any_sentinel(a[g][u]);
+#ifdef PCHAIN_TPROF
+    if (spins == 0 && pl.t_first == 0) pl.t_first = wall_clock64();
+    pl.polls++;
+#endif
     if (!__any(bad && aok) || pl.dead) break;
     if (spin_tick(spins, pl.ctl, pl.code, pl.dead)) break;
     pl.sleep();
   }
 multiply:
+#ifdef PCHAIN_TPROF
+  pl.t_ok = wall_clock64();
+  if (pl.t_first == 0) pl.t_first = pl.t_ok;
+#endif
   if constexpr (AMap::sum) {
 #pragma unroll
     for (int u = 0; u < NCH; ++u)
@@ -447,6 +469,9 @@
   float v[1];
   reduce_tiles<1, NW>(acc, red, v);
 #ifdef PCHAIN_TPROF
+  pl.t_red = wall_clock64();
+#endif
+#if defined(PCHAIN_TPROF) && !defined(VRNN_STATIC_TPROF)
   if (a_polled && pl.nap == 1) {
     const unsigned long long t3 = wall_clock64();
     pl.tp[0] += 1; pl.tp[1] += pl.t_first - t0; pl.tp[2] += pl.t_ok - pl.t_first; pl.tp[3] += t3 - pl.t_ok; pl.tp[4] += pl.polls;
@@ -526,6 +551,51 @@
   o.mu_p[oo] = mp; o.sd_p[oo] = sp; o.mu_q[oo] = mq; o.sd_q[oo] = sqc;
   o.raw_p[oo] = rp; o.raw_q[oo] = rq;
 }
+template <int NW, int OT, int NCH>
+__device__ __forceinline__ void tile_head_packed(const float* P, const float* Q, const float* bp, const float* bq, const float* eps, const HeadOut& o, int Z,
+                                                 int residual, float beta, float inv_beta, float sd_eps, int r0, int c0, int B, float* red, Poll& pl,
+                                                 const WRegs<OT, 2, NCH>& ws) {
+  const int t = threadIdx.x & 255;
+  const int row = r0 + (t >> 4), col = c0 + (t & 7);
+  const bool own = threadIdx.x < 256 && row < B && (t & 8) == 0;
+  const size_t oc = (size_t)(row < B ? row : r0) * Z + col;
+  float b0 = 0.f, b1 = 0.f, b2 = 0.f, b3 = 0.f, e = 0.f;
+  auto prefetch = [&]() { b0 = bp[col]; b1 = bp[Z + col]; b2 = bq[col]; b3 = bq[Z + col]; e = eps[oc]; };
+  f32x4 acc[2] = {{0.f, 0.f, 0.f, 0.f}, {0.f, 0.f, 0.f, 0.f}};
+  {
+    const float* const As[2] = {P, Q};
+    product_regs<NW, OT, 2, 2, MapId, NCH, false>(As, r0, B, NCH * 16 * NW, ws.w, acc, pl, prefetch);
+  }
+  float v[2];
+  reduce_tiles<2, NW>(acc, red, v);
+#ifdef PCHAIN_TPROF
+  pl.t_red = wall_clock64();
+#endif
+  const float s0 = __builtin_bit_cast(float, __builtin_amdgcn_update_dpp(0, __builtin_bit_cast(int, v[0]), 0x128, 0xf, 0xf, false));
+  const float s1 = __builtin_bit_cast(float, __builtin_amdgcn_update_dpp(0, __builtin_bit_cast(int, v[1]), 0x128, 0xf, 0xf, false));
+  if (!own) return;
+  const size_t oo = (size_t)row * Z + col;
+  const float mp = v[0] + b0, rp = s0 + b1, rq = s1 + b3;
+  float mq = v[1] + b2;
+  const float sp = softplus_beta(rp, beta, inv_beta) + sd_eps;
+  const float sq = softplus_beta(rq, beta, inv_beta) + sd_eps;
+  if (o.muq_raw != nullptr) o.muq_raw[oo] = mq;
+  float sqc = sq;
+  if (residual == 1) {
+    mq += mp;
+  } else if (residual == 2) {
+    const float pq = 1.f / (sq * sq), pp = 1.f / (sp * sp);
+    const float var = 1.f / (pq + pp);
+    mq = var * (mq * pq + mp * pp);
+    sqc = sqrtf(var);
+  } else if (residual == 3) {
+    mq = mp;
+    sqc = sp;
+  }
+  put(o.z, r0, c0 & ~15, row, col, e * sqc + mq);
+  o.mu_p[oo] = mp; o.sd_p[oo] = sp; o.mu_q[oo] = mq; o.sd_q[oo] = sqc;
+  o.raw_p[oo] = rp; o.raw_q[oo] = rq;
+}
 
 template <int NW, int OT = OP_F32, class WS = WMem>
 __device__ __forceinline__ void tile_gru(const float* X, int ldx, bool polled, const float* Wih, int K, const float* xg, const float* bih,
@@ -558,8 +628,16 @@
   }
   float v[3];
   reduce_tiles<3, NW>(acc, red, v);
+#ifdef PCHAIN_TPROF
+  pl.t_red = wall_clock64();
+#endif
   if (threadIdx.x >= 256) return;
-  if (__any(own && (is_sentinel(w[0]) | is_sentinel(w[1]) | is_sentinel(w[2]) | is_sentinel(w[3])))) poll_words<4>(ps, po, w, own, pl);
+  if (__any(own && (is_sentinel(w[0]) | is_sentinel(w[1]) | is_sentinel(w[2]) | is_sentinel(w[3])))) {
+#ifdef PCHAIN_TPROF
+    pl.late++;
+#endif
+    poll_words<4>(ps, po, w, own, pl);
+  }
   if (!own) return;
   const float r = sigmoidf_(v[0] + x0 + w[0]);
   const float u = sigmoidf_(v[1] + x1 + w[1]);
@@ -618,7 +696,17 @@
         acc[0] = a1[0];
       }
     }
-    reduce_tiles<2, NW>(acc, red, v);
+    if constexpr (WS::products == 1) {
+      f32x4 a1[1] = {acc[0]};
+      float v1[1];
+      reduce_tiles<1, NW>(a1, red, v1);
+      v[0] = v1[0];
+    } else {
+      reduce_tiles<2, NW>(acc, red, v);
+    }
+#ifdef PCHAIN_TPROF
+  pl.t_red = wall_clock64();
+#endif
   } else {
     prefetch();
   }
@@ -698,6 +786,9 @@
     const int la[2] = {0, 0}, cs[2] = {c0, c0};
     tile_product<NW, OT, 2, 2, MapId>(ws, As, la, true, r0, B, Ws, cs, K, acc, pl, prefetch);
     reduce_tiles<2, NW>(acc, red, v);
+#ifdef PCHAIN_TPROF
+  pl.t_red = wall_clock64();
+#endif
   }
   if (threadIdx.x >= 256) return;
   if (a.has_gin && __any(own && is_sentinel(g0))) {
diff --git a/benchmarking-lvms_amd/csrc/vrnn_static.h b/benchmarking-lvms_amd/csrc/vrnn_static.h
--- a/benchmarking-lvms_amd/csrc/vrnn_static.h
+++ b/benchmarking-lvms_amd/csrc/vrnn_static.h
@@ -54,13 +54,23 @@
   return d;
 }
 
-constexpr std::initializer_list<int> kFwdResident = {1, 2, 3, 4, 5};
+constexpr std::initializer_list<int> kFwdResident = {1, 2, 4, 5};
 constexpr std::initializer_list<int> kBwdResident = {0, 1, 2, 3, 5, 6, 7, 8, 9};
 inline bool one_tile_each(const Program& p, std::initializer_list<int> links) {
   for (int i : links)
     if (tiles_per_workgroup((p.B + 15) / 16, p.d[i].ct, p.d[i].nwg, p.xcd != 0) > 1) return false;
   return true;
 }
+constexpr int kFwdGentleTiles = 6, kBwdGentleTiles = 2;
+inline bool gentle_fits(const Program& p, int link, int max_tiles) {
+  return tiles_per_workgroup((p.B + 15) / 16, p.d[link].ct, p.d[link].nwg, p.xcd != 0) <= max_tiles;
+}
+
+inline LinkRange head_deal(int ctZ, int rt, int g, bool xcd) {
+  LinkRange r{2 * ctZ, 0, range_for(2 * ctZ * rt, g)};
+  if (r.nwg > g || tiles_per_workgroup(rt, r.ct, r.nwg, xcd) > 1) r.nwg = 0;
+  return r;
+}
 
 }
 }
diff --git a/benchmarking-lvms_amd/csrc/vrnn_static.hip b/benchmarking-lvms_amd/csrc/vrnn_static.hip
--- a/benchmarking-lvms_amd/csrc/vrnn_static.hip
+++ b/benchmarking-lvms_amd/csrc/vrnn_static.hip
@@ -1,6 +1,9 @@
 #include <algorithm>
 #include <mutex>
 
+#ifdef VRNN_STATIC_TPROF
+#define PCHAIN_TPROF
+#endif
 #include "common.h"
 #include "pchain.h"
 #include "vrnn_static.h"
@@ -16,8 +19,9 @@
 };
 
 constexpr int kMaxTiles = 8;
-__device__ __forceinline__ int tile_lanes(int w, int wg0, int nwg, int rt, int ct, bool xcd) {
-  TileIter it(w, wg0, nwg, rt, ct, xcd);
+__device__ __forceinline__ int tile_lanes(int w, int wg0, int nwg, int rt, int ct, int xcd) {
+  asm volatile("" : "+s"(xcd));
+  TileIter it(w, wg0, nwg, rt, ct, xcd != 0);
   const int lane = threadIdx.x & 63;
   it.j += lane * it.step;
   return (lane < kMaxTiles && it.valid()) ? (it.r0() | (it.c() << 16)) : -1;
@@ -35,7 +39,7 @@
 __global__ __launch_bounds__(NW * 64, 1) void static_lin_chain_kernel(LinChainArgs a) {
   __shared__ __attribute__((aligned(16))) float red[2][NW * 256];
   const int w = blockIdx.x, B = a.B;
-  const int tiles = tile_lanes(w, a.wg0, a.nwg, (B + 15) / 16, a.ct, a.xcd != 0);
+  const int tiles = tile_lanes(w, a.wg0, a.nwg, (B + 15) / 16, a.ct, a.xcd);
   const int nt = tile_count(tiles);
   if (nt == 0) return;
   Poll pl{a.ctl, 0u, false, 1};
@@ -106,12 +110,35 @@
 struct Deal {
   int wg0, nwg, ct, s_begin, s_end, idx;
 };
-
+__device__ __forceinline__ bool idle(const Deal& d, int s, int nt) {
+  asm volatile("" : "+s"(nt));
+  return nt == 0 || s < d.s_begin || s >= d.s_end;
+}
+
+#ifdef VRNN_STATIC_TPROF
+constexpr int kTprofKinds = 10, kTprofSlots = 8, kTprofRole = kTprofKinds * kTprofSlots;
+#define TP_VISIT(kind, ...) do { wk.tp_begin(); __VA_ARGS__; wk.tp_end(kind); } while (0)
+#else
+#define TP_VISIT(kind, ...) __VA_ARGS__
+#endif
 struct Walk {
   float* red0;
   float* red1;
   int par, B;
   Poll pl;
+#ifdef VRNN_STATIC_TPROF
+  unsigned long long* tp;
+  unsigned long long t0;
+  __device__ __forceinline__ void tp_begin() { pl.t_first = pl.t_ok = pl.t_red = 0; pl.late = 0; t0 = wall_clock64(); }
+  __device__ __forceinline__ void tp_end(int kind) {
+    if (threadIdx.x != 0) return;
+    const unsigned long long t = wall_clock64();
+    unsigned long long* c = tp + kind * kTprofSlots;
+    c[5] += t - t0;
+    if (pl.t_ok == 0) { c[6] += 1; return; }
+    c[0] += 1; c[1] += pl.t_first - t0; c[2] += pl.t_ok - pl.t_first; c[3] += pl.t_red - pl.t_ok; c[4] += t - pl.t_red; c[7] += pl.late;
+  }
+#endif
   __device__ __forceinline__ float* red() { par ^= 1; return par ? red0 : red1; }
   __device__ __forceinline__ void at(const Deal& d, int s, bool gentle, unsigned li = 0) {
     pl.nap = gentle ? 16 : 1;
@@ -141,13 +168,14 @@
 #pragma unroll
   for (int li = 1; li < N; ++li) load_lin<NW, K>(r.rest[li - 1], q.W[li], K, tiles, nt);
 }
-template <int NW>
-__device__ __forceinline__ void load_head(Res<kH, 4>& r, const HeadArgs& q, int tiles, int nt) {
+__device__ __forceinline__ int tile_c0_head(int tiles) { return (__builtin_amdgcn_readlane(tiles, 0) >> 16) * 8; }
+template <int NW>
+__device__ __forceinline__ void load_head(Res<kH, 2>& r, const HeadArgs& q, int tiles, int nt) {
   if (nt == 0) return;
-  const int c0 = tile_c0(tiles);
-  const float* const Ws[4] = {q.Wp, q.Wp, q.Wq, q.Wq};
-  const int cs[4] = {c0, q.Z + c0, c0, q.Z + c0};
-  load_w<NW, OP_F32, 4, 1>(r.w, Ws, cs, kH);
+  const int c0 = tile_c0_head(tiles);
+  const float* const Ws[2] = {q.Wp, q.Wq};
+  const int lo[2] = {c0, c0}, hi[2] = {q.Z + c0, q.Z + c0};
+  load_w_packed<NW, OP_F32, 2, 1>(r.w, Ws, lo, hi, kH);
 }
 template <int NW>
 __device__ __forceinline__ void load_gru(Res<kH, 3>& r, const GruArgs& q, int tiles, int nt) {
@@ -166,9 +194,9 @@
   load_w<NW, OP_F32, 2, 1>(r.w, Ws, cs, kH);
 }
 
-template <int NW, int K, int FLAGS, class WS>
-__device__ __forceinline__ void visit_lin(const LinArgs& q, const Deal& d, int s, int tiles, int nt, Walk& wk, const WS& ws) {
-  if (nt == 0 || s < d.s_begin || s >= d.s_end) return;
+template <int NW, int K, int FLAGS>
+__device__ __forceinline__ void visit_lin(const LinArgs& q, const Deal& d, int s, int tiles, int nt, Walk& wk, const Res<K>& ws) {
+  if (idle(d, s, nt)) return;
   constexpr bool sum3 = (FLAGS & DF_A_SUM3) != 0;
   wk.at(d, s, (FLAGS & DF_GENTLE) != 0);
   const float* A = q.a.at(s);
@@ -178,16 +206,43 @@
     return LinLate{q.bias, q.add.at(s), q.gate.at(s), q.ld1, q.ld2, (FLAGS & DF_ADD_POLLED) != 0, (FLAGS & DF_RELU) != 0, q.slope,
                    Out{q.orm.at(s), q.ld3, (FLAGS & DF_RM_SC1) != 0, q.o16.at(s), q.n16, q.o16b.at(s), q.n16b}};
   };
-  for (int tk = 0; tk < (WS::resident ? 1 : nt); ++tk) {
+  const int trc = __builtin_amdgcn_readlane(tiles, 0), tr0 = trc & 0xffff, tc0 = (trc >> 16) * 16;
+  tile_lin_late<NW, OP_F32>(A, q.ld0, true, q.W, K, late, tr0, tc0, wk.B, wk.red(), wk.pl, A2, A3, q.w_width, ws);
+}
+
+template <int NW, int K, int MAXT>
+__device__ __forceinline__ void load_gentle(Res<K> (&r)[MAXT], const float* W, int tiles) {
+  const float* const Ws[1] = {W};
+#pragma unroll
+  for (int tk = 0; tk < MAXT; ++tk) {
+    const int trc = __builtin_amdgcn_readlane(tiles, tk);
+    if (trc < 0) break;
+    const int cs[1] = {(trc >> 16) * 16};
+    load_w<NW, OP_F32, 1, K / 256>(r[tk].w, Ws, cs, K);
+  }
+}
+template <int NW, int K, int FLAGS, int MAXT>
+__device__ __forceinline__ void visit_gentle(const LinArgs& q, const Deal& d, int s, int tiles, Walk& wk, const Res<K> (&ws)[MAXT]) {
+  if (s < d.s_begin || s >= d.s_end) return;
+  wk.at(d, s, true);
+  const float* A = q.a.at(s);
+  auto late = [&]() {
+    return LinLate{q.bias, q.add.at(s), q.gate.at(s), q.ld1, q.ld2, (FLAGS & DF_ADD_POLLED) != 0, (FLAGS & DF_RELU) != 0, q.slope,
+                   Out{q.orm.at(s), q.ld3, (FLAGS & DF_RM_SC1) != 0, q.o16.at(s), q.n16, q.o16b.at(s), q.n16b}};
+  };
+  asm volatile("" : "+v"(tiles));
+#pragma unroll
+  for (int tk = 0; tk < MAXT; ++tk) {
     const int trc = __builtin_amdgcn_readlane(tiles, tk), tr0 = trc & 0xffff, tc0 = (trc >> 16) * 16;
+    if (trc < 0) break;
     if constexpr ((FLAGS & DF_CANARY) != 0) canary_wait(A, tr0, K, wk.pl, q.ld0);
-    tile_lin_late<NW, OP_F32>(A, q.ld0, true, q.W, K, late, tr0, tc0, wk.B, wk.red(), wk.pl, A2, A3, q.w_width, ws);
+    tile_lin_late<NW, OP_F32>(A, q.ld0, true, q.W, K, late, tr0, tc0, wk.B, wk.red(), wk.pl, nullptr, nullptr, q.w_width, ws[tk]);
   }
 }
 
 template <int NW, int N, int K0, int K, bool GATED>
 __device__ __forceinline__ void visit_run(const SeqArgs& q, const Deal& d, int s, int tiles, int nt, Walk& wk, const RunRes<N, K0, K>& rr) {
-  if (nt == 0 || s < d.s_begin || s >= d.s_end) return;
+  if (idle(d, s, nt)) return;
   const int trc = __builtin_amdgcn_readlane(tiles, 0), tr0 = trc & 0xffff, tc0 = (trc >> 16) * 16;
   const float* A = q.a0.at(s);
 #pragma unroll
@@ -205,19 +260,19 @@
 }
 
 template <int NW>
-__device__ __forceinline__ void visit_head(const HeadArgs& q, const Deal& d, int s, int tiles, int nt, Walk& wk, const Res<kH, 4>& ws) {
-  if (nt == 0 || s < d.s_begin || s >= d.s_end) return;
+__device__ __forceinline__ void visit_head(const HeadArgs& q, const Deal& d, int s, int tiles, int nt, Walk& wk, const Res<kH, 2>& ws) {
+  if (idle(d, s, nt)) return;
   wk.at(d, s, false);
   const HeadOut o{q.mu_p.at(s), q.sd_p.at(s), q.mu_q.at(s), q.sd_q.at(s), q.raw_p.at(s), q.raw_q.at(s), q.muq_raw.at(s),
                   Out{q.z.at(s), q.ld3, false, q.z16.at(s), q.n16, q.z16b.at(s), q.n16b}};
   const int trc = __builtin_amdgcn_readlane(tiles, 0);
-  tile_head<NW, OP_F32>(q.P.at(s), q.Q.at(s), true, q.Wp, q.bp, q.Wq, q.bq, q.eps.at(s), o, kH, q.Z, q.residual, q.beta, q.inv_beta, q.sd_eps,
-                        trc & 0xffff, (trc >> 16) * 16, wk.B, wk.red(), wk.pl, ws);
+  tile_head_packed<NW, OP_F32>(q.P.at(s), q.Q.at(s), q.bp, q.bq, q.eps.at(s), o, q.Z, q.residual, q.beta, q.inv_beta, q.sd_eps, trc & 0xffff,
+                               (trc >> 16) * 8, wk.B, wk.red(), wk.pl, ws);
 }
 
 template <int NW>
 __device__ __forceinline__ void visit_gru(const GruArgs& q, const Deal& d, int s, int tiles, int nt, Walk& wk, const Res<kH, 3>& ws) {
-  if (nt == 0 || s < d.s_begin || s >= d.s_end) return;
+  if (idle(d, s, nt)) return;
   wk.at(d, s, false);
   const Out o{q.hrm.at(s), q.ld3, true, q.h16.at(s), q.n16, q.h16b.at(s), q.n16b};
   const int trc = __builtin_amdgcn_readlane(tiles, 0);
@@ -227,7 +282,7 @@
 
 template <int NW>
 __device__ __forceinline__ void visit_dz(const DzArgs& q, const Deal& d, int s, int tiles, int nt, Walk& wk, const Res<kH>& ws) {
-  if (nt == 0 || s < d.s_begin || s >= d.s_end) return;
+  if (idle(d, s, nt)) return;
   wk.at(d, s, false);
   DzIn z;
   z.mu_q = q.mu_q.at(s); z.sd_q = q.sd_q.at(s); z.mu_p = q.mu_p.at(s); z.sd_p = q.sd_p.at(s); z.eps = q.eps.at(s); z.raw_q = q.raw_q.at(s);
@@ -244,7 +299,7 @@
 
 template <int NW>
 __device__ __forceinline__ void visit_grub(const GrubArgs& q, const Deal& d, int s, int tiles, int nt, Walk& wk, const Res<kH, 2>& ws) {
-  if (nt == 0 || s < d.s_begin || s >= d.s_end) return;
+  if (idle(d, s, nt)) return;
   wk.at(d, s, false);
   GrubIn g;
   g.D0 = q.D0.at(s); g.D1 = q.D1.at(s); g.W0 = q.W0; g.W1 = q.W1; g.g_in = q.g_in.at(s); g.g_add = q.g_add.at(s); g.ld_gadd = q.ld1;
@@ -265,6 +320,23 @@
   return *(const A*)p;
 }
 
+#ifdef VRNN_STATIC_TPROF
+__device__ __forceinline__ void tp_open(Walk& wk, unsigned long long* lds) {
+  if (threadIdx.x < kTprofRole) lds[threadIdx.x] = 0;
+  __syncthreads();
+  wk.tp = lds;
+}
+__device__ __forceinline__ void tp_flush(const Walk& wk, unsigned long long* prof, int role, bool chosen) {
+  if (threadIdx.x != 0 || !chosen || prof == nullptr) return;
+  for (int i = 0; i < kTprofRole; ++i) prof[role * kTprofRole + i] = wk.tp[i];
+}
+#define TP_OPEN() __shared__ unsigned long long tp_lds[kTprofRole]; tp_open(wk, tp_lds)
+#define TP_FLUSH(role, chosen) tp_flush(wk, a.prof, role, chosen)
+#else
+#define TP_OPEN()
+#define TP_FLUSH(role, chosen)
+#endif
+
 struct FwdArgs {
   LinArgs hproj;
   SeqArgs run[2];
@@ -274,17 +346,20 @@
   Deal deal[6];
   int B, s0, S, xcd;
   Ctl ctl;
+#ifdef VRNN_STATIC_TPROF
+  unsigned long long* prof;
+#endif
 };
 constexpr int kFwdProducts = 4, kBwdProducts = 2;
 
 template <int NW, int HALF>
-__device__ __forceinline__ void fwd_half(const FwdArgs& a, int w, int rt, bool xcd, Walk& wk) {
+__device__ __forceinline__ void fwd_half(const FwdArgs& a, int w, int rt, int xcd, Walk& wk) {
   const int t1 = tile_lanes(w, a.deal[1 + HALF].wg0, a.deal[1 + HALF].nwg, rt, a.deal[1 + HALF].ct, xcd), n1 = tile_count(t1);
   const int t3 = tile_lanes(w, a.deal[3].wg0, a.deal[3].nwg, rt, a.deal[3].ct, xcd), n3 = tile_count(t3);
   const int t4 = tile_lanes(w, a.deal[4].wg0, a.deal[4].nwg, rt, a.deal[4].ct, xcd), n4 = tile_count(t4);
   const int t5 = tile_lanes(w, a.deal[5].wg0, a.deal[5].nwg, rt, a.deal[5].ct, xcd), n5 = tile_count(t5);
   RunRes<3, kR, kH> run;
-  Res<kH, 4> head;
+  Res<kH, 2> head;
   RunRes<4, kH, kH> phi;
   Res<kH, 3> gru;
   load_run<NW>(run, kargs<FwdArgs>().run[HALF], t1, n1);
@@ -292,23 +367,29 @@
   load_run<NW>(phi, kargs<FwdArgs>().phi, t4, n4);
   load_gru<NW>(gru, kargs<FwdArgs>().gru, t5, n5);
   for (int s = a.s0; s < a.S; ++s) {
-    visit_run<NW, 3, kR, kH, false>(kargs<FwdArgs>().run[HALF], kargs<FwdArgs>().deal[1 + HALF], s, t1, n1, wk, run);
-    visit_head<NW>(kargs<FwdArgs>().head, kargs<FwdArgs>().deal[3], s, t3, n3, wk, head);
-    visit_run<NW, 4, kH, kH, false>(kargs<FwdArgs>().phi, kargs<FwdArgs>().deal[4], s, t4, n4, wk, phi);
-    visit_gru<NW>(kargs<FwdArgs>().gru, kargs<FwdArgs>().deal[5], s, t5, n5, wk, gru);
-  }
+    TP_VISIT(1 + HALF, visit_run<NW, 3, kR, kH, false>(kargs<FwdArgs>().run[HALF], kargs<FwdArgs>().deal[1 + HALF], s, t1, n1, wk, run));
+    TP_VISIT(3, visit_head<NW>(kargs<FwdArgs>().head, kargs<FwdArgs>().deal[3], s, t3, n3, wk, head));
+    TP_VISIT(4, visit_run<NW, 4, kH, kH, false>(kargs<FwdArgs>().phi, kargs<FwdArgs>().deal[4], s, t4, n4, wk, phi));
+    TP_VISIT(5, visit_gru<NW>(kargs<FwdArgs>().gru, kargs<FwdArgs>().deal[5], s, t5, n5, wk, gru));
+  }
+  TP_FLUSH(HALF, w == a.deal[1 + HALF].wg0);
 }
 
 template <int NW>
 __global__ __launch_bounds__(NW * 64, 1) void vrnn_static_fwd_kernel(FwdArgs a) {
   extern __shared__ __attribute__((aligned(16))) float lds_red[];
   const int w = blockIdx.x, rt = (a.B + 15) / 16;
-  const bool xcd = a.xcd != 0;
+  const int xcd = a.xcd;
   Walk wk{lds_red, lds_red + kFwdProducts * NW * 256, 0, a.B, Poll{a.ctl, 0u, false, 1}};
+  TP_OPEN();
   if (w >= a.deal[0].wg0) {
     const int t0 = tile_lanes(w, a.deal[0].wg0, a.deal[0].nwg, rt, a.deal[0].ct, xcd), n0 = tile_count(t0);
     if (n0 == 0) return;
-    for (int s = a.s0; s < a.S; ++s) visit_lin<NW, kR, DF_RM_SC1 | DF_GENTLE | DF_CANARY>(kargs<FwdArgs>().hproj, kargs<FwdArgs>().deal[0], s, t0, n0, wk, WMem());
+    Res<kR> hproj[kFwdGentleTiles];
+    load_gentle<NW, kR>(hproj, kargs<FwdArgs>().hproj.W, t0);
+    for (int s = a.s0; s < a.S; ++s)
+      TP_VISIT(0, visit_gentle<NW, kR, DF_RM_SC1 | DF_GENTLE | DF_CANARY>(kargs<FwdArgs>().hproj, kargs<FwdArgs>().deal[0], s, t0, wk, hproj));
+    TP_FLUSH(2, w == a.deal[0].wg0);
     return;
   }
   if (w < a.deal[2].wg0) fwd_half<NW, 0>(a, w, rt, xcd, wk);
@@ -324,10 +405,13 @@
   Deal deal[10];
   int B, s0, S, xcd;
   Ctl ctl;
+#ifdef VRNN_STATIC_TPROF
+  unsigned long long* prof;
+#endif
 };
 
 template <int NW, int HALF>
-__device__ __forceinline__ void bwd_half(const BwdArgs& a, int w, int rt, bool xcd, Walk& wk) {
+__device__ __forceinline__ void bwd_half(const BwdArgs& a, int w, int rt, int xcd, Walk& wk) {
   const int t0 = tile_lanes(w, a.deal[0].wg0, a.deal[0].nwg, rt, a.deal[0].ct, xcd), n0 = tile_count(t0);
   const int t1 = tile_lanes(w, a.deal[1 + HALF].wg0, a.deal[1 + HALF].nwg, rt, a.deal[1 + HALF].ct, xcd), n1 = tile_count(t1);
   const int t5 = tile_lanes(w, a.deal[5].wg0, a.deal[5].nwg, rt, a.deal[5].ct, xcd), n5 = tile_count(t5);
@@ -346,34 +430,40 @@
   load_lin<NW, kH>(dz, kargs<BwdArgs>().dz.WT, kH, t7, n7);
   load_run<NW>(run, kargs<BwdArgs>().run[HALF], t8, n8);
   for (int s = a.s0; s < a.S; ++s) {
-    visit_grub<NW>(kargs<BwdArgs>().grub, kargs<BwdArgs>().deal[0], s, t0, n0, wk, grub);
-    visit_lin<NW, kR, 0>(kargs<BwdArgs>().part[HALF], kargs<BwdArgs>().deal[1 + HALF], s, t1, n1, wk, part);
-    visit_lin<NW, kH, DF_A_SUM3>(kargs<BwdArgs>().sum, kargs<BwdArgs>().deal[5], s, t5, n5, wk, sum);
-    visit_run<NW, 2, kH, kH, true>(kargs<BwdArgs>().phi, kargs<BwdArgs>().deal[6], s, t6, n6, wk, phi);
-    visit_dz<NW>(kargs<BwdArgs>().dz, kargs<BwdArgs>().deal[7], s, t7, n7, wk, dz);
-    visit_run<NW, 3, 2 * kH, kH, true>(kargs<BwdArgs>().run[HALF], kargs<BwdArgs>().deal[8 + HALF], s, t8, n8, wk, run);
-  }
+    TP_VISIT(0, visit_grub<NW>(kargs<BwdArgs>().grub, kargs<BwdArgs>().deal[0], s, t0, n0, wk, grub));
+    TP_VISIT(1 + HALF, visit_lin<NW, kR, 0>(kargs<BwdArgs>().part[HALF], kargs<BwdArgs>().deal[1 + HALF], s, t1, n1, wk, part));
+    TP_VISIT(5, visit_lin<NW, kH, DF_A_SUM3>(kargs<BwdArgs>().sum, kargs<BwdArgs>().deal[5], s, t5, n5, wk, sum));
+    TP_VISIT(6, visit_run<NW, 2, kH, kH, true>(kargs<BwdArgs>().phi, kargs<BwdArgs>().deal[6], s, t6, n6, wk, phi));
+    TP_VISIT(7, visit_dz<NW>(kargs<BwdArgs>().dz, kargs<BwdArgs>().deal[7], s, t7, n7, wk, dz));
+    TP_VISIT(8 + HALF, visit_run<NW, 3, 2 * kH, kH, true>(kargs<BwdArgs>().run[HALF], kargs<BwdArgs>().deal[8 + HALF], s, t8, n8, wk, run));
+  }
+  TP_FLUSH(HALF, w == a.deal[1 + HALF].wg0);
 }
 
 template <int NW>
 __global__ __launch_bounds__(NW * 64, 1) void vrnn_static_bwd_kernel(BwdArgs a) {
   extern __shared__ __attribute__((aligned(16))) float lds_red[];
   const int w = blockIdx.x, rt = (a.B + 15) / 16;
-  const bool xcd = a.xcd != 0;
+  const int xcd = a.xcd;
   Walk wk{lds_red, lds_red + kBwdProducts * NW * 256, 0, a.B, Poll{a.ctl, 0u, false, 1}};
+  TP_OPEN();
   if (w >= a.deal[3].wg0) {
     const int t = tile_lanes(w, a.deal[3].wg0, a.deal[3].nwg, rt, a.deal[3].ct, xcd), n = tile_count(t);
     if (n == 0) return;
     Res<kR> part;
     load_lin<NW, kR>(part, kargs<BwdArgs>().part[2].W, kargs<BwdArgs>().part[2].w_width, t, n);
-    for (int s = a.s0; s < a.S; ++s) visit_lin<NW, kR, 0>(kargs<BwdArgs>().part[2], kargs<BwdArgs>().deal[3], s, t, n, wk, part);
+    for (int s = a.s0; s < a.S; ++s) TP_VISIT(3, visit_lin<NW, kR, 0>(kargs<BwdArgs>().part[2], kargs<BwdArgs>().deal[3], s, t, n, wk, part));
+    TP_FLUSH(3, w == a.deal[3].wg0);
     return;
   }
   if (w >= a.deal[4].wg0) {
     const int t = tile_lanes(w, a.deal[4].wg0, a.deal[4].nwg, rt, a.deal[4].ct, xcd), n = tile_count(t);
     if (n == 0) return;
+    Res<3 * kR> gb[kBwdGentleTiles];
+    load_gentle<NW, 3 * kR>(gb, kargs<BwdArgs>().gb.W, t);
     for (int s = a.s0; s < a.S; ++s)
-      visit_lin<NW, 3 * kR, DF_ADD_POLLED | DF_RM_SC1 | DF_GENTLE | DF_CANARY>(kargs<BwdArgs>().gb, kargs<BwdArgs>().deal[4], s, t, n, wk, WMem());
+      TP_VISIT(4, visit_gentle<NW, 3 * kR, DF_ADD_POLLED | DF_RM_SC1 | DF_GENTLE | DF_CANARY>(kargs<BwdArgs>().gb, kargs<BwdArgs>().deal[4], s, t, wk, gb));
+    TP_FLUSH(2, w == a.deal[4].wg0);
     return;
   }
   if (w < a.deal[2].wg0) bwd_half<NW, 0>(a, w, rt, xcd, wk);
@@ -475,11 +565,15 @@
       !shaped(d[3], K_HEAD, 0, kH) || !shaped(d[4], K_LINSEQ, DF_RELU, kH) || !shaped(d[5], K_GRU, 0, kH))
     return 1;
   if (!run(d[1], 3, kR) || !run(d[2], 3, kR) || !run(d[4], 4, 0)) return 1;
-  if (!one_tile_each(p, kFwdResident)) return 1;
+  if (!one_tile_each(p, kFwdResident) || !gentle_fits(p, 0, kFwdGentleTiles)) return 1;
   const int half = d[2].wg0, gentle = d[0].wg0;
   if (d[1].wg0 != 0 || !within(d[1], 0, half) || !within(d[2], half, gentle) || d[0].nwg <= 0) return 1;
   for (int i = 3; i < 6; ++i)
     if (!within(d[i], 0, gentle)) return 1;
+  const Desc& hd = d[3];
+  if (hd.i[HEAD_I_Z] != kH || hd.ct * 16 != kH) return 1;
+  const LinkRange heads = head_deal(hd.ct, (p.B + 15) / 16, gentle, p.xcd != 0);
+  if (heads.nwg <= 0 || (p.xcd && heads.nwg % 8 != 0)) return 1;
   FwdArgs a{};
   a.hproj = lin_args(p, d[0]);
   a.run[0] = seq_args(p, d[1]); a.run[1] = seq_args(p, d[2]); a.phi = seq_args(p, d[4]);
@@ -493,7 +587,11 @@
                   g.n16[N16_OUTB], g.i[GRU_I_R]};
   int grid = 0;
   for (int i = 0; i < 6; ++i) { a.deal[i] = deal_of(d[i], i); grid = std::max(grid, d[i].wg0 + d[i].nwg); }
+  a.deal[3].wg0 = heads.wg0; a.deal[3].nwg = heads.nwg; a.deal[3].ct = heads.ct;
   a.B = p.B; a.s0 = p.s_first; a.S = S; a.xcd = p.xcd; a.ctl = p.ctl;
+#ifdef VRNN_STATIC_TPROF
+  a.prof = pchain_profile_buffer();
+#endif
   const size_t lds = sizeof(float) * 2 * kFwdProducts * 16 * 256;
   BLVM_TRY(static_go(&vrnn_static_fwd_kernel<16>, 0, grid, lds, "vrnn_static_fwd"));
   hipLaunchKernelGGL(vrnn_static_fwd_kernel<16>, dim3(grid), dim3(1024), lds, stream, a);
@@ -514,7 +612,7 @@
       !shaped(d[9], K_LINSEQ, DF_SEQ_GATE, kH))
     return 1;
   if (!run(d[6], 2, 0) || !run(d[8], 3, 2 * kH) || !run(d[9], 3, 2 * kH)) return 1;
-  if (!one_tile_each(p, kBwdResident) || d[7].p[DZ_D2_16] != nullptr) return 1;
+  if (!one_tile_each(p, kBwdResident) || !gentle_fits(p, 4, kBwdGentleTiles) || d[7].p[DZ_D2_16] != nullptr) return 1;
   const int half = d[2].wg0, gentle = d[4].wg0, spare = d[3].wg0;
   if (!within(d[1], 0, half) || !within(d[8], 0, half) || !within(d[2], half, gentle) || !within(d[9], half, gentle) || !within(d[4], gentle, spare) ||
       d[3].nwg <= 0)
@@ -539,6 +637,9 @@
   int grid = 0;
   for (int i = 0; i < 10; ++i) { a.deal[i] = deal_of(d[i], i); grid = std::max(grid, d[i].wg0 + d[i].nwg); }
   a.B = p.B; a.s0 = p.s_first; a.S = S; a.xcd = p.xcd; a.ctl = p.ctl;
+#ifdef VRNN_STATIC_TPROF
+  a.prof = pchain_profile_buffer() ? pchain_profile_buffer() + 256 : nullptr;
+#endif
   const size_t lds = sizeof(float) * 2 * kBwdProducts * 16 * 256;
   BLVM_TRY(static_go(&vrnn_static_bwd_kernel<16>, 1, grid, lds, "vrnn_static_bwd"));
   hipLaunchKernelGGL(vrnn_static_bwd_kernel<16>, dim3(grid), dim3(1024), lds, stream, a);
```

Result: no change. 81.05 million (median of 6 runs) (+0.6%).
